# XuyangBai/D3Feat

Hardware: AMD Instinct MI355X
Metric: fragments/sec (30k-pt clouds) (higher is better)
Workload: dtype f32; 1 GPU; SURVEY §8d config #2: synthetic 3DMatch room fragment, 300k raw pts -> grid subsample 0.03 m (~29k pts per cloud) -> self-pair -> 5-level pyramid -> full KPFCNN forward (random-init weights (reference initialiser, seed 42), 14.1M params)...; points_per_cloud=29369, fragments_per_gpu=2141, parallelism=fragment-dp1, fragments_per_replay=12, engine_fallbacks=0, engine_isolated_replays=0

## Files before the change

### d3feat_amd/_lib.py

```python
import ctypes as C
import os

_HERE = os.path.dirname(os.path.abspath(__file__))
LIB_PATH = os.environ.get("D3FEAT_AMD_LIB") or os.path.join(_HERE, "lib", "libd3feat_amd.so")

D3F_OK = 0
ERRORS = {-1: "HIP runtime / kernel launch failure", -2: "workspace too small", -3: "invalid argument"}
ST_EMPTY_ELEMENT, ST_NEG_CELL, ST_KEY_RANGE, ST_HIT_OVERFLOW, ST_OUT_OVERFLOW, ST_KEY_WIDTH = 1, 2, 4, 8, 16, 32
PAD_NUM_SUPPORTS = -2147483648
NEIGHBOR_CAP = 1024
MAX_BATCH = 255
TOPK_MAX = 8192
PAIRS_KMAX = 1024
REPEAT_COUNTS_MAX = 16
MATCH_KMAX = 8192
VALIDATION_NMAX = 1024
SCENES_MAX = 256
GRID_RESET_MAX = 8
VP_INDEX_RANGE, VP_COUNT_RANGE = 1, 2

_vp, _sz, _i, _f = C.c_void_p, C.c_size_t, C.c_int, C.c_float

SIGNATURES = {
    "d3f_version": (_i, []),
    "d3f_trace_marker": (_i, [_i, _vp]),
    "d3f_pack_status": (_i, [_vp, _vp, _i, _vp, _i, _vp, _i, _vp, _i, _vp, _i, _i, _i, _vp]),
    "d3f_grid_subsample_workspace_bytes": (_sz, [_i, _i, _i, _i]),
    "d3f_batch_grid_subsample": (_i, [_vp, _i, _vp, _i, _f, _vp, _i, _vp, _i, _vp, _vp, _vp, _vp, _vp, _vp, _sz, _vp]),
    "d3f_batch_grid_subsample_async": (_i, [_vp, _i, _vp, _i, _f, _vp, _i, _i, _i, _vp, _vp, _vp, _sz, _vp]),
    "d3f_batch_grid_subsample_async_inplace": (_i, [_vp, _i, _vp, _i, _f, _vp, _i, _i, _vp, _vp, _vp, _sz, _vp]),
    "d3f_stack_self_pair": (_i, [_vp, _i, _vp, _i, _vp, _vp, _vp, _vp]),
    "d3f_radius_neighbors_workspace_bytes": (_sz, [_i, _i, _i]),
    "d3f_batch_radius_neighbors": (_i, [_vp, _i, _vp, _i, _vp, _vp, _i, _f, _vp, _i, _i, _i, _vp, _vp, _sz, _vp]),
    "d3f_neighbor_grid_bytes": (_sz, [_i, _i]),
    "d3f_neighbor_grid_order_offset": (_sz, [_i, _i]),
    "d3f_neighbor_grid_build": (_i, [_vp, _i, _vp, _i, _f, _vp, _sz, _vp]),
    "d3f_neighbor_grid_boxed_form": (_i, [_i, _i]),
    "d3f_geometry_reset": (_i, [_vp, _i, _vp, _vp, _vp, _vp, _i, _vp]),
    "d3f_neighbor_grid_build_boxed": (_i, [_vp, _i, _vp, _i, _f, _vp, _vp, _sz, _vp]),
    "d3f_stack_self_pair_boxed": (_i, [_vp, _i, _vp, _i, _vp, _vp, _vp, _vp, _vp, _vp]),
    "d3f_batch_grid_subsample_async_boxed": (_i, [_vp, _vp, _i, _vp, _i, _f, _vp, _i, _i, _i, _vp, _vp, _vp, _vp, _vp, _sz, _vp]),
    "d3f_neighbor_grid_search": (_i, [_vp, _sz, _i, _vp, _i, _vp, _i, _f, _i, _vp, _i, _i, _i, _i, _i, _f, _i, _vp, _vp]),
    "d3f_neighbor_grid_search_ordered": (_i, [_vp, _sz, _i, _vp, _i, _vp, _i, _f, _vp, _sz, _vp, _i, _i, _i, _i, _i, _f, _i, _vp, _vp]),
    "d3f_neighbor_grid_inv_offset": (_sz, [_i, _i]),
    "d3f_neighbor_grid_xyz_offset": (_sz, [_i, _i]),
    "d3f_row_positive": (_i, [_vp, _i, _i, _i, _vp, _vp, _i, _vp]),
    "d3f_kpconv_aggregate": (_i, [_vp, _i, _vp, _i, _vp, _i, _i, _vp, _i, _i, _vp, _vp, _i, _f, _i, _i, _vp, _vp, _vp, _vp,
                                  _vp, _i, _vp]),
    "d3f_kpconv_deform_aggregate": (_i, [_vp, _i, _vp, _i, _vp, _i, _i, _vp, _i, _i, _vp, _i, _f, _vp, _i, _i, _vp, _i, _f, _i, _i, _vp,
                                         _vp, _vp, _vp, _i, _vp]),
    "d3f_kpconv_fused_c1": (_i, [_vp, _i, _vp, _i, _vp, _i, _i, _vp, _i, _vp, _i, _f, _i, _i, _vp, _i, _vp, _vp, _vp, _i, _i,
                                 _f, _vp, _i, _vp, _vp, _vp, _i, _vp]),
    "d3f_kpconv_fused32": (_i, [_vp, _i, _vp, _i, _vp, _i, _i, _vp, _i, _vp, _vp, _i, _f, _i, _i, _vp, _vp, _vp, _vp, _i, _i, _f, _vp,
                                _i, _vp, _vp, _vp, _i, _vp]),
    "d3f_kpconv_fused_supported": (_i, [_i, _i, _i, _i, _i]),
    "d3f_kpconv_pack_weights": (_i, [_vp, _i, _i, _vp, _vp]),
    "d3f_kpconv_fused": (_i, [_vp, _i, _vp, _i, _vp, _i, _i, _vp, _i, _i, _vp, _vp, _i, _f, _i, _i, _vp, _i, _vp, _vp, _vp, _i, _i,
                              _f, _vp, _i, _vp, _vp, _vp, _i, _vp]),
    "d3f_kpconv_fused32_x3": (_i, [_vp, _i, _vp, _i, _vp, _i, _i, _vp, _i, _vp, _vp, _i, _f, _i, _i, _vp, _vp, _vp, _vp, _i, _i, _f, _vp,
                                   _i, _vp, _vp, _vp, _i, _vp]),
    "d3f_kpconv_packed_x3_bytes": (_sz, [_i, _i]),
    "d3f_kpconv_pack_weights_x3": (_i, [_vp, _i, _i, _vp, _vp]),
    "d3f_kpconv_fused_x3": (_i, [_vp, _i, _vp, _i, _vp, _i, _i, _vp, _i, _i, _vp, _vp, _i, _f, _i, _i, _vp, _i, _vp, _vp, _vp, _i, _i,
                                 _f, _vp, _i, _vp, _vp, _vp, _i, _vp]),
    "d3f_gemm_workspace_bytes": (_sz, [_i, _i, _i, _i]),
    "d3f_gemm_bf16_workspace_bytes": (_sz, [_i, _i, _i, _i]),
    "d3f_gemm_f32": (_i, [_vp, _i, _vp, _i, _vp, _i, _i, _i, _i, _vp, _vp, _vp, _vp, _i, _i, _f, _vp, _sz, _vp, _i, _vp]),
    "d3f_gemm_upsample_cat_f32": (_i, [_vp, _i, _i, _i, _vp, _i, _vp, _i, _i, _vp, _i, _vp, _i, _i, _i, _vp, _vp, _i, _f, _vp, _sz,
                                       _vp, _vp, _i, _vp]),
    "d3f_ind_max_pool": (_i, [_vp, _i, _i, _i, _vp, _i, _i, _i, _vp, _i, _vp, _vp, _vp, _vp, _i, _vp]),
    "d3f_closest_pool_cat": (_i, [_vp, _i, _i, _i, _vp, _i, _i, _vp, _i, _i, _vp, _i, _vp, _vp, _vp]),
    "d3f_affine_act": (_i, [_vp, _i, _i, _i, _vp, _vp, _vp, _i, _i, _f, _vp, _i, _vp, _vp]),
    "d3f_pack_descriptors": (_i, [_vp, _vp, _i, _i, _vp, _i, _vp, _i, _vp, _vp]),
    "d3f_pack_descriptors_to": (_i, [_vp, _vp, _i, _i, _vp, _i, _vp, _i, _vp, _vp, _i, _i, _i, _vp, _vp, _vp]),
    "d3f_topk_workspace_bytes": (_sz, [_i, _i, _i, _i]),
    "d3f_topk_records": (_i, [_vp, _i, _vp, _i, _i, _vp, _i, _i, _vp, _vp, _i, _i, _i, _vp, _i, _i, _vp, _i, _vp, _vp, _vp, _vp, _sz,
                              _vp]),
    "d3f_feature_nn_workspace_bytes": (_sz, [_i]),
    "d3f_feature_nn": (_i, [_vp, _i, _i, _vp, _i, _i, _i, _vp, _vp, _vp, _sz, _vp]),
    "d3f_mutual_matches_workspace_bytes": (_sz, [_i]),
    "d3f_mutual_matches": (_i, [_vp, _i, _vp, _i, _vp, _vp, _vp, _sz, _vp]),
    "d3f_ransac_hypotheses": (_i, [_vp, _i, _vp, _i, _vp, _i, _f, _f, C.c_uint64, C.c_uint64, _i, _vp, _vp, _vp]),
    "d3f_ransac_draw": (_i, [C.c_uint64, C.c_uint64, _i, _i]),
    "d3f_neighbor_grid_score": (_i, [_vp, _sz, _i, _vp, _i, _vp, _i, _f, _vp, _vp, _vp, _vp]),
    "d3f_register_pairs_workspace_bytes": (_sz, [_i, _i, _i, _i]),
    "d3f_register_pairs": (_i, [_vp, _i, _i, _i, _i, _vp, _vp, _i, _i, _f, _i, _f, _f, _i, _i, C.c_uint64, _vp, _f] + [_vp] * 11
                           + [_sz, _vp]),
    "d3f_repeatability_pairs": (_i, [_vp, _i, _i, _i, _vp, _vp, _i, _vp, _i, _vp, _vp, _i, _vp, _vp, _vp]),
    "d3f_match_pairs_workspace_bytes": (_sz, [_i, _vp, _i]),
    "d3f_match_pairs": (_i, [_vp, _i, _i, _i, _i, _vp, _vp, _i, _vp, _f, _vp, _i, _vp, _vp, _vp, _sz, _vp]),
    "d3f_register_pairs_counts_workspace_bytes": (_sz, [_i, _i, _i, _vp, _i, _i]),
    "d3f_register_pairs_counts": (_i, [_vp, _i, _i, _i, _i, _vp, _vp, _i, _vp, _i, _f, _i, _f, _f, _i, _i, C.c_uint64, _vp, _f] + [_vp] * 10
                                  + [_sz, _vp]),
    "d3f_overlap_pairs": (_i, [_vp, _sz, _i, _i, _vp, _i, _f, _vp, _vp, _i, _vp]),
    "d3f_validation_pairs_workspace_bytes": (_sz, [_i, _i]),
    "d3f_validation_pairs": (_i, [_vp, _i, _i, _vp, _i, _vp, _i, _i, _vp, _vp, _vp, _i, _vp, _i, _f, _i, _f, _f, _f, _f] + [_vp] * 5
                             + [_sz, _vp]),
    "d3f_loss_gradients_workspace_bytes": (_sz, [_i, _i, _i]),
    "d3f_loss_gradients": (_i, [_vp, _i, _i, _vp, _i, _vp, _i, _i, _vp, _vp, _vp, _i, _vp, _i, _f, _i, _f, _f, _f, _f, _i, _vp, _i, _vp, _i,
                                _vp, _vp, _vp, _sz, _vp]),
    "d3f_neighbor_transpose_workspace_bytes": (_sz, [_i, _i]),
    "d3f_neighbor_transpose": (_i, [_vp, _i, _i, _i, _vp, _i, _vp, _vp, _vp, _sz, _vp]),
    "d3f_detect_head_backward_workspace_bytes": (_sz, [_i, _i, _i]),
    "d3f_detect_head_backward": (_i, [_vp, _i, _i, _i, _vp, _i, _i, _vp, _vp, _i, _i, _vp, _vp, _vp, _i, _vp, _i, _vp, _i, _vp, _sz, _vp]),
    "d3f_pose_errors": (_i, [_vp, _vp, _i, _i, _vp, _vp, _vp, _vp, _vp, _vp]),
    "d3f_sanitize_descriptors": (_i, [_vp, _i, _i, _i, _i, _vp]),
    "d3f_matching_summary": (_i, [_vp, _vp, _vp, _i, _i, _vp, _i, _vp, _vp, _vp, _vp]),
    "d3f_registration_recall": (_i, [_vp, _i, _vp, _vp, _vp, _vp, _vp, _i, _i, _vp, _i, _vp, _vp, _vp, _vp, _vp]),
    "d3f_icp_pairs_workspace_bytes": (_sz, [_i, _i]),
    "d3f_icp_pairs": (_i, [_vp, _sz, _i, _vp, _i, _vp, _i, _vp, _vp, _i, _i] + [_vp] * 9 + [_sz, _vp]),
    "d3f_gemm_pack_bf16": (_i, [_vp, _i, _i, _i, _vp, _vp]),
    "d3f_gemm_pack_f32t": (_i, [_vp, _i, _i, _i, _vp, _vp]),
    "d3f_gemm_f32t": (_i, [_vp, _i, _i, _i, _vp, _i, _vp, _i, _i, _vp, _vp, _i, _i, _i, _vp, _vp, _vp, _vp, _i, _i, _f, _vp, _sz,
                           _vp, _vp, _i, _vp]),
    "d3f_gemm_x3_packed_bytes": (_sz, [_i, _i]),
    "d3f_gemm_pack_x3": (_i, [_vp, _i, _i, _i, _vp, _vp]),
    "d3f_gemm_x3_workspace_bytes": (_sz, [_i, _i, _i, _i]),
    "d3f_gemm_x3_plan": (_i, [_i, _i, _i, _i, _vp, _vp, _vp]),
    "d3f_gemm_x3_resident": (_i, [_i, _i, _i, _i]),
    "d3f_gemm_x3": (_i, [_vp, _i, _i, _i, _vp, _i, _vp, _i, _i, _vp, _vp, _i, _i, _i, _vp, _vp, _vp, _vp, _i, _i, _f, _vp, _sz,
                         _vp, _vp, _i, _vp]),
    "d3f_gemm_x3_gres": (_i, [_vp, _i, _i, _i, _vp, _i, _vp, _i, _i, _vp, _vp, _i, _i, _i, _vp, _vp, _vp, _vp, _i, _vp, _i, _i, _vp, _i, _f,
                              _vp, _sz, _vp, _vp, _i, _vp]),
    "d3f_gemm_bf16": (_i, [_vp, _i, _i, _i, _vp, _i, _vp, _i, _i, _vp, _vp, _i, _i, _i, _vp, _vp, _vp, _vp, _i, _i, _f, _vp, _sz,
                           _vp, _vp, _i, _i, _i, _vp]),
    "d3f_decode_xyz_records": (_i, [_vp, _i, _i, _i, _i, _i, _i, _i, _vp, _vp]),
    "d3f_detect_head": (_i, [_vp, _i, _i, _i, _vp, _i, _i, _vp, _vp, _i, _i, _vp, _i, _vp, _vp, _vp, _vp]),
}

_lib = None


class D3FeatLibraryError(RuntimeError):
    pass


def load():
    global _lib
    if _lib is not None:
        return _lib
    if not os.path.exists(LIB_PATH):
        raise D3FeatLibraryError(
            "d3feat_amd: %s not found -- the HIP extension is the only compute path. Build it with "
            "`python -c 'import __graft_entry__ as g; g.build()'` or `make -C d3feat_amd/csrc`." % LIB_PATH)
    lib = C.CDLL(LIB_PATH)
    for name, (res, args) in SIGNATURES.items():
        fn = getattr(lib, name)
        fn.restype = res
        fn.argtypes = args
    _lib = lib
    return lib


def check(rc, what):
    if rc != D3F_OK:
        raise D3FeatLibraryError("d3feat_amd.%s failed: %s (code %d)" % (what, ERRORS.get(rc, "unknown"), rc))
```

### d3feat_amd/csrc/gemm_common.h

```cpp
#pragma once
#include "common.h"
#include <type_traits>

typedef float f32x16 __attribute__((ext_vector_type(16)));

#define GM_BK 32

struct GemmGather {
    const int* gidx;
    int ld_gidx;
    int N1;
    const int* N1_dev;
    const float* A2;
    int lda2;
    int K1;
};

struct GemmEpi {
    const float* row_scale;
    const float* col_scale;
    const float* col_shift;
    const float* residual;
    int ldr;
    int leaky;
    float alpha;
    const int* ridx;
    int ld_ridx;
    int res_rows;
    const int* res_rows_dev;
};

__device__ __forceinline__ const float* gemm_residual_row(const GemmEpi& E, int m) {
    if (!E.ridx) return E.residual + (size_t)m * E.ldr;
    const int r = E.ridx[(size_t)m * E.ld_ridx];
    return (r >= 0 && r < d3f_dyn(E.res_rows, E.res_rows_dev)) ? E.residual + (size_t)r * E.ldr : nullptr;
}

__device__ __forceinline__ float gemm_epilogue(float v, int m, int n, const GemmEpi& E) {
    if (E.row_scale) v *= E.row_scale[m];
    if (E.col_scale) v *= E.col_scale[n];
    if (E.col_shift) v += E.col_shift[n];
    if (E.residual) v += E.residual[(size_t)m * E.ldr + n];
    if (E.leaky) v = v > 0.f ? v : v * E.alpha;
    return v;
}

__device__ __forceinline__ void gemm_tile_mfma(f32x16& acc, const float* as, const float* bs, int q0, int q1, int q2, int q3) {
    const int coff[4] = {q0, q1, q2, q3};
    float4 fa[4], fb[4];
#pragma unroll
    for (int q = 0; q < 4; ++q) {
        fa[q] = *(const float4*)&as[coff[q]];
        fb[q] = *(const float4*)&bs[coff[q]];
    }
    __builtin_amdgcn_sched_barrier(0);
#pragma unroll
    for (int q = 0; q < 4; ++q) {
#pragma unroll
        for (int e = 0; e < 4; ++e) {
            const float a = e == 0 ? fa[q].x : e == 1 ? fa[q].y : e == 2 ? fa[q].z : fa[q].w;
            const float b = e == 0 ? fb[q].x : e == 1 ? fb[q].y : e == 2 ? fb[q].z : fb[q].w;
            acc = __builtin_amdgcn_mfma_f32_32x32x2f32(b, a, acc, 0, 0, 0);
        }
    }
}

__global__ void __launch_bounds__(256)
gemm_splitk_reduce_kernel(const float* __restrict__ slab, int S, int M, int N, float* __restrict__ C, int ldc, GemmEpi E,
                          const int* __restrict__ M_dev, int res_bf16 = 0, int c_bf16 = 0) {
    const long long i = (long long)blockIdx.x * blockDim.x + threadIdx.x;
    if (i >= (long long)d3f_dyn(M, M_dev) * N) return;
    const int m = (int)(i / N), n = (int)(i % N);
    float v = 0.f;
    for (int s = 0; s < S; ++s) v += slab[((size_t)s * M + m) * N + n];
    if (res_bf16 && E.residual) {
        const float r = d3f_bf16_f32(((const unsigned short*)E.residual)[(size_t)m * E.ldr + n]);
        GemmEpi E2 = E;
        E2.residual = nullptr;
        E2.leaky = 0;
        v = gemm_epilogue(v, m, n, E2) + r;
        if (E.leaky) v = v > 0.f ? v : v * E.alpha;
    } else if (E.ridx && E.residual) {
        const float* rrow = gemm_residual_row(E, m);
        GemmEpi E2 = E;
        E2.residual = nullptr;
        E2.leaky = 0;
        v = gemm_epilogue(v, m, n, E2) + (rrow ? rrow[n] : 0.f);
        if (E.leaky) v = v > 0.f ? v : v * E.alpha;
    } else {
        v = gemm_epilogue(v, m, n, E);
    }
    if (c_bf16) ((unsigned short*)C)[(size_t)m * ldc + n] = (unsigned short)d3f_bf16_rne(v);
    else C[(size_t)m * ldc + n] = v;
}

static inline size_t gemm_slab_bytes(int S, int M, int N) { return S > 1 ? d3f_align((size_t)S * M * N * sizeof(float)) + 256 : 256; }

static inline int gemm_slab(int S, int M, int N, void* workspace, size_t workspace_bytes, float*& slab) {
    slab = nullptr;
    if (S > 1) {
        if (!workspace || workspace_bytes < (size_t)S * M * N * sizeof(float)) return D3F_ERR_WORKSPACE;
        slab = (float*)workspace;
    }
    return D3F_OK;
}

static inline void gemm_reduce(const float* slab, int S, int M, int N, float* C, int ldc, const GemmEpi& E, const int* M_dev,
                               hipStream_t stream, int res_bf16 = 0, int c_bf16 = 0) {
    if (S > 1)
        gemm_splitk_reduce_kernel<<<d3f_cdiv((long long)M * N, 256), 256, 0, stream>>>(slab, S, M, N, C, ldc, E, M_dev, res_bf16, c_bf16);
}

static inline int gemm_check_composite(bool f32_io, int kmul, unsigned a_mask, int M, int N, int N1, int C1, int C2, int lda, int ldc,
                                       int lds, int ldr, int ld_idx, const void* A, const void* W, const void* C, const int* idx,
                                       const void* skip, const void* residual, const float* col_scale, const float* col_shift,
                                       bool& empty) {
    const int q = f32_io ? 4 : 1;
    empty = false;
    if (M < 0 || N < 1 || N1 < 0 || C1 < 4 || C2 < 0 || (C1 % 4) || (C2 % 4) || (N % q) || lda < C1 || (lda % 4) || ldc < N || (ldc % q) ||
        (C2 > 0 && (lds < C2 || (lds % 4))) || (residual && (ldr < N || (ldr % q))) || (idx && ld_idx < 1) || (!idx && N1 < M))
        return D3F_ERR_ARG;
    if (((C1 + C2) % kmul) || (C2 > 0 && (C1 % kmul))) return D3F_ERR_ARG;
    empty = M == 0;
    if (empty) return D3F_OK;
    if (!A || !W || !C || (C2 > 0 && !skip) || ((uintptr_t)W & 15) || (((uintptr_t)A | (uintptr_t)skip) & a_mask)) return D3F_ERR_ARG;
    if (f32_io && (((uintptr_t)C | (uintptr_t)residual | (uintptr_t)col_scale | (uintptr_t)col_shift) & 15)) return D3F_ERR_ARG;
    return D3F_OK;
}

template <class F> static inline void gemm_with_epi(const GemmEpi& E, F&& f) {
    switch ((E.row_scale ? 1 : 0) | (E.residual ? 2 : 0)) {
    case 0: f(std::integral_constant<int, 0>{}); break;
    case 1: f(std::integral_constant<int, 1>{}); break;
    case 2: f(std::integral_constant<int, 2>{}); break;
    default: f(std::integral_constant<int, 3>{}); break;
    }
}

static inline void gemm_plan(int M, int N, int K, int M_hint, int& bm, int& bn, int& S, int& tps) {
    if (M_hint > 0 && M_hint < M) M = M_hint;
    auto blocks_of = [&](int m, int n) { return (long long)d3f_cdiv(M, m) * d3f_cdiv(N, n); };
    if (N <= 32) { bm = 128; bn = 32; }
    else { bm = 64; bn = 64; }
    const long long blocks = blocks_of(bm, bn);
    const int nt = d3f_cdiv(K, GM_BK);
    S = 1;
    if (blocks < 768 && nt > 16) {
        long long want = (1536 + blocks - 1) / blocks;
        long long maxs = nt / 8;
        S = (int)(want < maxs ? want : maxs);
        if (S > 64) S = 64;
        if (S < 1) S = 1;
    }
    tps = d3f_cdiv(nt, S);
    S = d3f_cdiv(nt, tps);
}
```

### d3feat_amd/csrc/gemm_f32.hip

```cpp
#include "gemm_common.h"
#include <cstdio>
#include <cstdlib>

#define GM_SA (GM_BK + 1)

template <int WM, int WN>
__global__ void __launch_bounds__(256)
gemm_f32_kernel(const float* __restrict__ A, int lda, const float* __restrict__ B, int ldb, float* __restrict__ C, int ldc,
                int M, int N, int K, int vecA, int vecB, int tiles_per_split, float* __restrict__ slab, GemmEpi E,
                const int* __restrict__ M_dev, GemmGather G) {
    constexpr int BM = 32 * WM, BN = 32 * WN;
    constexpr int A_F4 = BM * GM_BK / 4 / 256;
    constexpr int B_F4 = GM_BK * BN / 4 / 256;
    static_assert(WM * WN == 4 && A_F4 >= 1 && B_F4 >= 1, "tile shape");
    const int Mcap = M;
    M = d3f_dyn(M, M_dev);
    if ((int)(blockIdx.z * BM) >= M) return;
    __shared__ float As[2][BM * GM_SA];
    __shared__ __attribute__((aligned(16))) float Bs[2][GM_BK * BN];

    const int tid = threadIdx.x, lane = tid & 63, wave = tid >> 6;
    const int wm = wave / WN, wn = wave % WN;
    const int m0 = blockIdx.z * BM, n0 = blockIdx.x * BN;
    const int nt_all = (K + GM_BK - 1) / GM_BK;
// ... 381 lines not shown
    if (int rc = gemm_check_composite(true, 4, 15, M, N, N1, C1, C2, lda, ldc, lds, ldr, ld_idx, A, Wt, C, idx, skip, residual,
                                      col_scale, col_shift, empty))
        return rc;
    if (empty) return D3F_OK;
    const int Kp = (K + GD_BK - 1) / GD_BK * GD_BK;
    int bm, bn, S, tps;
    gemm_plan(M, N, K, M_hint, bm, bn, S, tps);
    float* slab;
    if (int rc = gemm_slab(S, M, N, workspace, workspace_bytes, slab)) return rc;
    GemmEpi E{row_scale, col_scale, col_shift, residual, ldr, leaky, alpha};
    GemmGather G{idx, ld_idx, N1, N1_dev, C2 > 0 ? skip : nullptr, lds, C1};
    static_assert((size_t)GD_STAGES * (128 + 32) * GD_BK * sizeof(float) <= 65536, "the ring needs an LDS opt-in (d3f_opt_in_lds)");
    const size_t lds_bytes = (size_t)GD_STAGES * (bm + bn) * GD_BK * sizeof(float);
    const long long items_cap = (long long)d3f_cdiv(N, bn) * S * d3f_cdiv(M, bm);
    const long long gsz = (items_cap + 7) / 8 * 8;
    if (gsz > 0x7fffffffll) return D3F_ERR_ARG;
    const dim3 grid((unsigned)gsz, 1, 1);
    gemm_with_epi(E, [&](auto epi) {
        constexpr int EPI = decltype(epi)::value;
        if (bn == 32) gemm_dma_kernel<4, 1, EPI><<<grid, 256, lds_bytes, stream>>>(A, lda, Wt, Kp, C, ldc, M, N, K, tps, S, slab, E, M_dev, G);
        else gemm_dma_kernel<2, 2, EPI><<<grid, 256, lds_bytes, stream>>>(A, lda, Wt, Kp, C, ldc, M, N, K, tps, S, slab, E, M_dev, G);
    });
    gemm_reduce(slab, S, M, N, C, ldc, E, M_dev, stream);
    D3F_LAUNCH_CHECK();
    return D3F_OK;
}

typedef __bf16 gb_bf16x8 __attribute__((ext_vector_type(8)));
#define GB_BK 32
#define GB_LS 40

__device__ __forceinline__ unsigned gb_pack2(float a, float b) { return d3f_bf16_rne(a) | (d3f_bf16_rne(b) << 16); }

__global__ void __launch_bounds__(256) gemm_pack_bf16_kernel(const float* __restrict__ B, int ldb, int K, int N, int Kp,
                                                             unsigned short* __restrict__ Wt) {
    const long long t = (long long)blockIdx.x * blockDim.x + threadIdx.x;
    if (t >= (long long)N * Kp) return;
    const int n = (int)(t / Kp), k = (int)(t % Kp);
    Wt[t] = (unsigned short)(k < K ? d3f_bf16_rne(B[(size_t)k * ldb + n]) : 0u);
}

extern "C" int d3f_gemm_pack_bf16(const float* B, int ldb, int K, int N, void* Wt, void* stream_) {
    hipStream_t stream = (hipStream_t)stream_;
    if (K < 1 || N < 1 || ldb < N || !B || !Wt) return D3F_ERR_ARG;
    const int Kp = (K + GB_BK - 1) / GB_BK * GB_BK;
    gemm_pack_bf16_kernel<<<d3f_cdiv((long long)N * Kp, 256), 256, 0, stream>>>(B, ldb, K, N, Kp, (unsigned short*)Wt);
    D3F_LAUNCH_CHECK();
    return D3F_OK;
}

template <bool ABF, bool CBF>
__global__ void __launch_bounds__(256)
gemm_bf16_kernel(const float* __restrict__ A, int lda, const unsigned short* __restrict__ Wt, int Kp, float* __restrict__ C,
                 int ldc, int M, int N, int K, int tiles_per_split, float* __restrict__ slab, GemmEpi E,
                 const int* __restrict__ M_dev, GemmGather G) {
    constexpr int BM = 64, BN = 64;
    const int Mcap = M;
    M = d3f_dyn(M, M_dev);
    if ((int)(blockIdx.z * BM) >= M) return;
    const unsigned gx_ = gridDim.x, gxy_ = gridDim.x * gridDim.y;
    const unsigned T_ = d3f_xcd_tile(blockIdx.x + gx_ * blockIdx.y + gxy_ * blockIdx.z, gxy_ * (unsigned)((M + BM - 1) / BM));
    const unsigned bz = T_ / gxy_, by = (T_ % gxy_) / gx_, bx = T_ % gx_;
    __shared__ __attribute__((aligned(16))) unsigned short As[2][BM * GB_LS];
    __shared__ __attribute__((aligned(16))) unsigned short Bs[2][BN * GB_LS];
    const int tid = threadIdx.x, lane = tid & 63, wave = tid >> 6;
    const int wm = wave >> 1, wn = wave & 1;
    const int m0 = bz * BM, n0 = bx * BN;
    const int nt_all = Kp / GB_BK;
    const int t_begin = by * tiles_per_split;
    const int t_end = min(nt_all, t_begin + tiles_per_split);
    int srow[2];
    {
        const int n1 = d3f_dyn(G.N1, G.N1_dev);
#pragma unroll
        for (int i = 0; i < 2; ++i) {
            const int gm = m0 + ((tid + i * 256) >> 3);
            int sr = gm < M ? gm : -1;
            if (G.gidx && sr >= 0) {
                sr = G.gidx[(size_t)gm * G.ld_gidx];
                if (sr < 0 || sr >= n1) sr = -1;
            }
            srow[i] = sr;
        }
    }
    const int brow = n0 + (tid >> 2);
    float4 ra[2];
    uint2 rh[2];
    uint4 rb;
    const unsigned short* Ah = (const unsigned short*)A;
    const unsigned short* A2h = (const unsigned short*)G.A2;
    auto load_tile = [&](int t) {
        const int k0 = t * GB_BK;
#pragma unroll
        for (int i = 0; i < 2; ++i) {
            const int e = tid + i * 256;
            const int gm = m0 + (e >> 3), k = k0 + ((e & 7) << 2);
            if (ABF) {
                uint2 v = make_uint2(0u, 0u);
                if (gm < M && k < K) {
                    if (G.A2 && k >= G.K1) v = *(const uint2*)(A2h + (size_t)gm * G.lda2 + (k - G.K1));
                    else if (srow[i] >= 0) v = *(const uint2*)(Ah + (size_t)srow[i] * lda + k);
                }
                rh[i] = v;
            } else {
                float4 v = make_float4(0.f, 0.f, 0.f, 0.f);
                if (gm < M && k < K) {
                    if (G.A2 && k >= G.K1) v = *(const float4*)(G.A2 + (size_t)gm * G.lda2 + (k - G.K1));
                    else if (srow[i] >= 0) v = *(const float4*)(A + (size_t)srow[i] * lda + k);
                }
                ra[i] = v;
            }
        }
        rb = (brow < N) ? *(const uint4*)(Wt + (size_t)brow * Kp + k0 + ((tid & 3) << 3)) : make_uint4(0u, 0u, 0u, 0u);
    };
    auto store_tile = [&](int buf) {
#pragma unroll
        for (int i = 0; i < 2; ++i) {
            const int e = tid + i * 256;
            const uint2 p = ABF ? rh[i] : make_uint2(gb_pack2(ra[i].x, ra[i].y), gb_pack2(ra[i].z, ra[i].w));
            *(uint2*)&As[buf][(e >> 3) * GB_LS + ((e & 7) << 2)] = p;
        }
        *(uint4*)&Bs[buf][(tid >> 2) * GB_LS + ((tid & 3) << 3)] = rb;
    };
    f32x16 acc;
#pragma unroll
    for (int r = 0; r < 16; ++r) acc[r] = 0.f;
    if (t_begin < t_end) {
        load_tile(t_begin);
        store_tile(0);
        __syncthreads();
        for (int t = t_begin; t < t_end; ++t) {
            const int buf = (t - t_begin) & 1;
            if (t + 1 < t_end) load_tile(t + 1);
            const unsigned short* ap = &As[buf][(32 * wm + (lane & 31)) * GB_LS + ((lane >> 5) << 3)];
            const unsigned short* bp = &Bs[buf][(32 * wn + (lane & 31)) * GB_LS + ((lane >> 5) << 3)];
            const uint4 a0 = *(const uint4*)ap, a1 = *(const uint4*)(ap + 16);
            const uint4 b0 = *(const uint4*)bp, b1 = *(const uint4*)(bp + 16);
            acc = __builtin_amdgcn_mfma_f32_32x32x16_bf16(__builtin_bit_cast(gb_bf16x8, a0), __builtin_bit_cast(gb_bf16x8, b0), acc, 0, 0, 0);
            acc = __builtin_amdgcn_mfma_f32_32x32x16_bf16(__builtin_bit_cast(gb_bf16x8, a1), __builtin_bit_cast(gb_bf16x8, b1), acc, 0, 0, 0);
            if (t + 1 < t_end) store_tile(buf ^ 1);
            __syncthreads();
        }
    }
    const int gn = n0 + 32 * wn + (lane & 31);
    if (gn >= N) return;
    float cs = 1.f, ch = 0.f;
    if (!slab) { cs = E.col_scale ? E.col_scale[gn] : 1.f; ch = E.col_shift ? E.col_shift[gn] : 0.f; }
#pragma unroll
    for (int r = 0; r < 16; ++r) {
        const int gm = m0 + 32 * wm + (r & 3) + 8 * (r >> 2) + 4 * (lane >> 5);
        if (gm >= M) continue;
        if (slab) { slab[((size_t)by * Mcap + gm) * N + gn] = acc[r]; continue; }
        float v = acc[r];
        if (E.row_scale) v *= E.row_scale[gm];
        v = v * cs + ch;
        if (E.residual)
            v += ABF ? d3f_bf16_f32(((const unsigned short*)E.residual)[(size_t)gm * E.ldr + gn]) : E.residual[(size_t)gm * E.ldr + gn];
        if (E.leaky) v = v > 0.f ? v : v * E.alpha;
        if (CBF) ((unsigned short*)C)[(size_t)gm * ldc + gn] = (unsigned short)d3f_bf16_rne(v);
        else C[(size_t)gm * ldc + gn] = v;
    }
}

static void gemm_bf16_split(int M, int N, int K, int M_hint, int& S, int& tps) {
    int bm, bn;
    gemm_plan(M, N > 32 ? N : 64, K, M_hint, bm, bn, S, tps);
    const int nt = ((K + GB_BK - 1) / GB_BK * GB_BK) / GB_BK;
    if (S > nt) S = nt;
    tps = d3f_cdiv(nt, S);
    S = d3f_cdiv(nt, tps);
}

extern "C" size_t d3f_gemm_bf16_workspace_bytes(int M, int N, int K, int M_hint) {
    if (M <= 0 || N <= 0 || K <= 0) return 256;
    int S, tps;
    gemm_bf16_split(M, N, K, M_hint, S, tps);
    return gemm_slab_bytes(S, M, N);
}

extern "C" int d3f_gemm_bf16(const void* A_, int N1, int lda, int C1, const int* idx, int ld_idx, const void* skip_, int lds,
                             int C2, const void* Wt, void* C_, int ldc, int M, int N, const float* row_scale,
                             const float* col_scale, const float* col_shift, const void* residual_, int ldr, int leaky,
                             float alpha, void* workspace, size_t workspace_bytes, const int* M_dev, const int* N1_dev,
                             int M_hint, int a_bf16, int c_bf16, void* stream_) {
    hipStream_t stream = (hipStream_t)stream_;
    const float* A = (const float*)A_;
    const float* skip = (const float*)skip_;
    const float* residual = (const float*)residual_;
    float* C = (float*)C_;
    const int K = C1 + C2;
    bool empty;
    if (int rc = gemm_check_composite(false, 4, a_bf16 ? 7 : 15, M, N, N1, C1, C2, lda, ldc, lds, ldr, ld_idx, A, Wt, C, idx, skip,
                                      residual, col_scale, col_shift, empty))
        return rc;
    if (empty) return D3F_OK;
    const int Kp = (K + GB_BK - 1) / GB_BK * GB_BK;
    int S, tps;
    gemm_bf16_split(M, N, K, M_hint, S, tps);
    float* slab;
    if (int rc = gemm_slab(S, M, N, workspace, workspace_bytes, slab)) return rc;
    if (d3f_cdiv(M, 64) > 65535) return D3F_ERR_ARG;
    GemmEpi E{row_scale, col_scale, col_shift, residual, ldr, leaky, alpha};
    GemmGather G{idx, ld_idx, N1, N1_dev, C2 > 0 ? skip : nullptr, lds, C1};
    dim3 grid(d3f_cdiv(N, 64), S, d3f_cdiv(M, 64));
#define D3F_GB(ABF_, CBF_) gemm_bf16_kernel<ABF_, CBF_><<<grid, 256, 0, stream>>>(A, lda, (const unsigned short*)Wt, Kp, C, ldc, M, N, K, tps, slab, E, M_dev, G)
    if (a_bf16) { if (c_bf16) D3F_GB(true, true); else D3F_GB(true, false); }
    else { if (c_bf16) D3F_GB(false, true); else D3F_GB(false, false); }
#undef D3F_GB
    gemm_reduce(slab, S, M, N, C, ldc, E, M_dev, stream, a_bf16, c_bf16);
    D3F_LAUNCH_CHECK();
    return D3F_OK;
}

#include "gemm_x3.h"

struct GemmX3Plan { int tn, waves, S, tps; };
static long long gemm_x3_cost(long long blocks, long long slots, int nt, int per_tile_x100, int& S) {
    long long best = -1;
    S = 1;
    for (int s = 1; s <= 64 && s * 4 <= nt; ++s) {
        const int t = d3f_cdiv(nt, s);
        if (d3f_cdiv(nt, t) != s) continue;
        const long long rounds = (blocks * s + slots - 1) / slots;
        const long long cost = rounds * (t + 12) * per_tile_x100 + (s > 1 ? 200ll * s : 0);
        if (best < 0 || cost < best) { best = cost; S = s; }
    }
    if (best < 0) best = ((blocks + slots - 1) / slots) * (nt + 12) * per_tile_x100;
    return best;
}
static GemmX3Plan gemm_x3_plan(int M, int N, int K, int M_hint) {
    if (M_hint > 0 && M_hint < M) M = M_hint;
    const int nt = K / GX_BK;
    GemmX3Plan p;
#ifdef D3F_GEMM_TUNING
    static const char* forced = getenv("D3F_X3_PLAN");
    if (forced) {
        int tn = 0, wv = 0, S = 0;
        if (sscanf(forced, "%d,%d,%d", &tn, &wv, &S) == 3 && ((tn == 1 && wv == 4) || (tn == 2 && wv == 4) || (tn == 4 && wv == 8)) && S >= 1 &&
            !(N <= 32 && tn != 1) && S * 4 <= (nt > 4 ? nt : 4)) {
            p.tn = tn; p.waves = wv; p.S = S < nt ? S : nt;
            p.tps = d3f_cdiv(nt, p.S);
            p.S = d3f_cdiv(nt, p.tps);
            return p;
        }
    }
#endif
    p.tn = N <= 32 ? 1 : 2;
    p.waves = 4;
    const long long c_small = gemm_x3_cost((long long)d3f_cdiv(M, 128) * d3f_cdiv(N, 32 * p.tn), 512, nt, 100, p.S);
    if (N >= 128) {
        int s_big;
        const long long c_big = gemm_x3_cost((long long)d3f_cdiv(M, 256) * d3f_cdiv(N, 128), 256, nt, 163, s_big);
        if (c_big < c_small) { p.tn = 4; p.waves = 8; p.S = s_big; }
    }
    p.tps = d3f_cdiv(nt, p.S);
    p.S = d3f_cdiv(nt, p.tps);
    return p;
}

extern "C" size_t d3f_gemm_x3_packed_bytes(int K, int N) {
    if (K < 1 || N < 1) return 0;
    return (size_t)d3f_cdiv(N, 32) * d3f_cdiv(K, GX_BK) * GX_CHUNK * sizeof(unsigned short);
}

extern "C" int d3f_gemm_pack_x3(const float* B, int ldb, int K, int N, void* Wx, void* stream_) {
    hipStream_t stream = (hipStream_t)stream_;
    if (K < 1 || N < 1 || ldb < N || !B || !Wx || ((uintptr_t)Wx & 15)) return D3F_ERR_ARG;
    const int nkt = d3f_cdiv(K, GX_BK);
    const long long total = (long long)d3f_cdiv(N, 32) * nkt * GX_CHUNK;
    gemm_pack_x3_kernel<<<d3f_cdiv(total, 256), 256, 0, stream>>>(B, ldb, K, N, nkt, total, (unsigned short*)Wx);
    D3F_LAUNCH_CHECK();
    return D3F_OK;
}

extern "C" int d3f_gemm_x3_plan(int M, int N, int K, int M_hint, int* rows, int* cols, int* slices) {
    if (M <= 0 || N <= 0 || K < GX_BK || (K % GX_BK)) return D3F_ERR_ARG;
    const GemmX3Plan p = gemm_x3_plan(M, N, K, M_hint);
    if (rows) *rows = 32 * p.waves;
    if (cols) *cols = 32 * p.tn;
    if (slices) *slices = p.S;
    return D3F_OK;
}

extern "C" size_t d3f_gemm_x3_workspace_bytes(int M, int N, int K, int M_hint) {
    if (M <= 0 || N <= 0 || K < GX_BK) return 256;
    const GemmX3Plan p = gemm_x3_plan(M, N, K, M_hint);
    return gemm_slab_bytes(p.S, M, N);
}

static size_t gemm_x3r_lds_bytes(int nkt, int NG) {
    return (size_t)nkt * NG * GX_CHUNK * sizeof(unsigned short) + GXR_PATCH_BYTES + GXR_EPI_BYTES;
}

extern "C" int d3f_gemm_x3_resident(int M, int N, int K, int M_hint) {
    if (N < 1 || K < GX_BK || (K % GX_BK)) return 0;
    const int NG = d3f_cdiv(N, 32), m_eff = (M_hint > 0 && M_hint < M) ? M_hint : M;
    return (NG == 1 || NG == 2 || NG == 4) && gemm_x3r_lds_bytes(K / GX_BK, NG) <= 160 * 1024 && m_eff >= 65536;
}

static int gemm_x3_run(const float* A, int N1, int lda, int C1, const int* idx, int ld_idx, const float* skip, int lds, int C2,
                       const void* Wx, float* C, int ldc, int M, int N, const float* row_scale, const float* col_scale,
                       const float* col_shift, const float* residual, int ldr, const int* res_idx, int ld_res_idx, int res_rows,
                       const int* res_rows_dev, int leaky, float alpha, void* workspace, size_t workspace_bytes, const int* M_dev,
                       const int* N1_dev, int M_hint, void* stream_) {
    hipStream_t stream = (hipStream_t)stream_;
    const int K = C1 + C2;
    bool empty;
    if (int rc = gemm_check_composite(true, GX_BK, 15, M, N, N1, C1, C2, lda, ldc, lds, ldr, ld_idx, A, Wx, C, idx, skip, residual,
                                      col_scale, col_shift, empty))
        return rc;
    if (res_idx && (ld_res_idx < 1 || res_rows < 0)) return D3F_ERR_ARG;
    if (empty) return D3F_OK;
    if (res_idx && !residual) return D3F_ERR_ARG;
    GemmEpi E{row_scale, col_scale, col_shift, residual, ldr, leaky, alpha, res_idx, ld_res_idx, res_rows, res_rows_dev};
    GemmGather G{idx, ld_idx, N1, N1_dev, C2 > 0 ? skip : nullptr, lds, C1};
    const int nkt = K / GX_BK, NG = d3f_cdiv(N, 32);
    if (!res_idx && d3f_gemm_x3_resident(M, N, K, M_hint)) {
        static std::atomic<int> cus_of[64];
        int dev = 0;
        if (hipGetDevice(&dev) != hipSuccess) return D3F_ERR_HIP;
        int cus = cus_of[dev & 63].load(std::memory_order_relaxed);
        if (!cus) {
            hipDeviceProp_t pr;
            if (hipGetDeviceProperties(&pr, dev) != hipSuccess) return D3F_ERR_HIP;
            cus = pr.multiProcessorCount > 0 ? pr.multiProcessorCount : 256;
            cus_of[dev & 63].store(cus, std::memory_order_relaxed);
        }
        static std::atomic<unsigned long long> lds_done{0};
        const void* const fns[3] = {(const void*)gemm_x3r_kernel<1>, (const void*)gemm_x3r_kernel<2>, (const void*)gemm_x3r_kernel<4>};
        if (d3f_opt_in_lds(lds_done, fns, 160 * 1024) != D3F_OK) return D3F_ERR_HIP;
        const int grid = std::min(cus, d3f_cdiv(d3f_cdiv(M, 32), 8));
#define D3F_GXR(TN_) gemm_x3r_kernel<TN_><<<grid, 512, gemm_x3r_lds_bytes(nkt, NG), stream>>>(A, lda, (const unsigned short*)Wx, nkt, C, ldc, M, N, E, M_dev, G)
        if (NG == 4) D3F_GXR(4);
        else if (NG == 2) D3F_GXR(2);
        else D3F_GXR(1);
#undef D3F_GXR
        D3F_LAUNCH_CHECK();
        return D3F_OK;
    }
    const GemmX3Plan pl = gemm_x3_plan(M, N, K, M_hint);
    const int S = pl.S, tps = pl.tps, bm = 32 * pl.waves;
    float* slab;
    if (int rc = gemm_slab(S, M, N, workspace, workspace_bytes, slab)) return rc;
    if (d3f_cdiv(M, bm) > 65535) return D3F_ERR_ARG;
    dim3 grid(d3f_cdiv(N, 32 * pl.tn), S, d3f_cdiv(M, bm));
#define D3F_GX(TN_, WV_) gemm_x3_kernel<TN_, WV_><<<grid, 64 * WV_, 0, stream>>>(A, lda, (const unsigned short*)Wx, nkt, NG, C, ldc, M, N, tps, slab, E, M_dev, G)
    if (pl.waves == 8) D3F_GX(4, 8);
    else if (pl.tn == 1) D3F_GX(1, 4);
    else D3F_GX(2, 4);
#undef D3F_GX
    gemm_reduce(slab, S, M, N, C, ldc, E, M_dev, stream);
    D3F_LAUNCH_CHECK();
    return D3F_OK;
}

extern "C" int d3f_gemm_x3(const float* A, int N1, int lda, int C1, const int* idx, int ld_idx, const float* skip, int lds, int C2,
                           const void* Wx, float* C, int ldc, int M, int N, const float* row_scale, const float* col_scale,
                           const float* col_shift, const float* residual, int ldr, int leaky, float alpha, void* workspace,
                           size_t workspace_bytes, const int* M_dev, const int* N1_dev, int M_hint, void* stream_) {
    return gemm_x3_run(A, N1, lda, C1, idx, ld_idx, skip, lds, C2, Wx, C, ldc, M, N, row_scale, col_scale, col_shift, residual, ldr,
                       nullptr, 0, 0, nullptr, leaky, alpha, workspace, workspace_bytes, M_dev, N1_dev, M_hint, stream_);
}

extern "C" int d3f_gemm_x3_gres(const float* A, int N1, int lda, int C1, const int* idx, int ld_idx, const float* skip, int lds, int C2,
                                const void* Wx, float* C, int ldc, int M, int N, const float* row_scale, const float* col_scale,
                                const float* col_shift, const float* residual, int ldr, const int* res_idx, int ld_res_idx,
                                int res_rows, const int* res_rows_dev, int leaky, float alpha, void* workspace, size_t workspace_bytes,
                                const int* M_dev, const int* N1_dev, int M_hint, void* stream_) {
    return gemm_x3_run(A, N1, lda, C1, idx, ld_idx, skip, lds, C2, Wx, C, ldc, M, N, row_scale, col_scale, col_shift, residual, ldr,
                       res_idx, ld_res_idx, res_rows, res_rows_dev, leaky, alpha, workspace, workspace_bytes, M_dev, N1_dev, M_hint,
                       stream_);
}
```

### d3feat_amd/csrc/gemm_x3.h

```cpp
#pragma once
#include "gemm_common.h"

#define GX_BK 32
#define GX_LS 40
#define GX_CHUNK (3 * 32 * GX_LS)

__device__ __forceinline__ unsigned gx_cvt_pk(float lo, float hi) {
    unsigned r;
    asm("v_cvt_pk_bf16_f32 %0, %1, %2" : "=v"(r) : "v"(lo), "v"(hi));
    return r;
}

typedef float gx_f4 __attribute__((ext_vector_type(4)));
__device__ __forceinline__ void gx_ld16(gx_f4& r, const void* p) { asm volatile("global_load_dwordx4 %0, %1, off" : "=v"(r) : "v"(p) : "memory"); }
template <int OFF> __device__ __forceinline__ void gx_ld16o(gx_f4& r, const void* p) {
    asm volatile("global_load_dwordx4 %0, %1, off offset:%2" : "=v"(r) : "v"(p), "n"(OFF) : "memory");
}

__device__ __forceinline__ float gx_sub(float a, float b) {
    float r;
    asm("v_sub_f32 %0, %1, %2" : "=v"(r) : "v"(a), "v"(b));
    return r;
}
__device__ __forceinline__ void gx_split8(const gx_f4& x0, const gx_f4& x1, uint4 (&pl)[3]) {
    const float v[8] = {x0[0], x0[1], x0[2], x0[3], x1[0], x1[1], x1[2], x1[3]};
    unsigned p[3][4];
#pragma unroll
    for (int i = 0; i < 4; ++i) {
        float a = v[2 * i], b = v[2 * i + 1];
        p[0][i] = gx_cvt_pk(a, b);
        a = gx_sub(a, __uint_as_float(p[0][i] << 16));
        b = gx_sub(b, __uint_as_float(p[0][i] & 0xffff0000u));
        p[1][i] = gx_cvt_pk(a, b);
        a = gx_sub(a, __uint_as_float(p[1][i] << 16));
        b = gx_sub(b, __uint_as_float(p[1][i] & 0xffff0000u));
        p[2][i] = gx_cvt_pk(a, b);
    }
#pragma unroll
    for (int s = 0; s < 3; ++s) pl[s] = make_uint4(p[s][0], p[s][1], p[s][2], p[s][3]);
}

__global__ void __launch_bounds__(256) gemm_pack_x3_kernel(const float* __restrict__ B, int ldb, int K, int N, int nkt, long long total,
                                                           unsigned short* __restrict__ Wx) {
    const long long t = (long long)blockIdx.x * blockDim.x + threadIdx.x;
    if (t >= total) return;
    const int kk = (int)(t % GX_LS);
    long long q = t / GX_LS;
    const int r = (int)(q % 32); q /= 32;
    const int p = (int)(q % 3); q /= 3;
    const int kt = (int)(q % nkt);
    const int ng = (int)(q / nkt);
    const int k = kt * GX_BK + kk, n = ng * 32 + r;
    unsigned out = 0u;
    if (kk < GX_BK && k < K && n < N) {
        float w = B[(size_t)k * ldb + n];
        unsigned h = d3f_bf16_rne(w);
        if (p > 0) { w -= __uint_as_float(h << 16); h = d3f_bf16_rne(w); }
        if (p > 1) { w -= __uint_as_float(h << 16); h = d3f_bf16_rne(w); }
        out = h;
    }
    Wx[t] = (unsigned short)out;
}

template <int NB, int STRIDE>
__device__ __forceinline__ void gx_dma_round(const void* sbase, unsigned dst, const unsigned (&vo)[4]) {
    unsigned keep;
    if constexpr (NB == 2)
        asm volatile("s_mov_b32 %0, m0\n\ts_mov_b32 m0, %2\n\ts_nop 0\n\tglobal_load_lds_dwordx4 %3, %1\n\t"
                     "s_add_u32 m0, m0, %5\n\ts_nop 0\n\tglobal_load_lds_dwordx4 %4, %1\n\ts_mov_b32 m0, %0"
                     : "=&s"(keep) : "s"(sbase), "s"(dst), "v"(vo[0]), "v"(vo[1]), "n"(STRIDE) : "memory", "scc");
    else if constexpr (NB == 4)
        asm volatile("s_mov_b32 %0, m0\n\ts_mov_b32 m0, %2\n\ts_nop 0\n\tglobal_load_lds_dwordx4 %3, %1\n\t"
                     "s_add_u32 m0, m0, %7\n\ts_nop 0\n\tglobal_load_lds_dwordx4 %4, %1\n\t"
                     "s_add_u32 m0, m0, %7\n\ts_nop 0\n\tglobal_load_lds_dwordx4 %5, %1\n\t"
                     "s_add_u32 m0, m0, %7\n\ts_nop 0\n\tglobal_load_lds_dwordx4 %6, %1\n\ts_mov_b32 m0, %0"
                     : "=&s"(keep) : "s"(sbase), "s"(dst), "v"(vo[0]), "v"(vo[1]), "v"(vo[2]), "v"(vo[3]), "n"(STRIDE) : "memory", "scc");
    else static_assert(NB < 0, "add the round");
}

template <int TN, int WAVES>
__global__ void __launch_bounds__(64 * WAVES) __attribute__((amdgpu_waves_per_eu(2, 2)))
gemm_x3_kernel(const float* __restrict__ A, int lda, const unsigned short* __restrict__ Wx, int nkt, int NG, float* __restrict__ C,
               int ldc, int M, int N, int tiles_per_split, float* __restrict__ slab, GemmEpi E, const int* __restrict__ M_dev,
               GemmGather G) {
    constexpr int BM = 32 * WAVES, BN = 32 * TN, NTH = 64 * WAVES;
    constexpr int NB = (480 * TN + NTH - 1) / NTH;
    constexpr int SB = NB * NTH * 16;
    constexpr int WAITN = 4 + NB;
    static_assert((TN == 1 || TN == 2 || TN == 4) && (WAVES == 4 || WAVES == 8), "tile shape");
    const int Mcap = M;
    M = d3f_dyn(M, M_dev);
    if ((int)(blockIdx.z * BM) >= M) return;
    const unsigned gx_ = gridDim.x, gxy_ = gridDim.x * gridDim.y;
    const unsigned T_ = d3f_xcd_tile(blockIdx.x + gx_ * blockIdx.y + gxy_ * blockIdx.z, gxy_ * (unsigned)((M + BM - 1) / BM));
    const unsigned bz = T_ / gxy_, by = (T_ % gxy_) / gx_, bx = T_ % gx_;
    __shared__ __attribute__((aligned(16))) unsigned char Bs[3 * SB];
    const int tid = threadIdx.x, lane = tid & 63, wave = tid >> 6;
    const int m0 = bz * BM, n0 = bx * BN;
    const int t_begin = by * tiles_per_split;
    const int t_end = min(nkt, t_begin + tiles_per_split);
    const int t_last = t_end - 1;

    const int gm_a = m0 + 32 * wave + (lane & 31);
    const float* arow = gd_zero_line;
    const float* a2row = gd_zero_line;
    unsigned amask = 0u, a2mask = 0u;
    if (gm_a < M) {
        int sr = gm_a;
        if (G.gidx) {
            const int n1 = d3f_dyn(G.N1, G.N1_dev);
            sr = G.gidx[(size_t)gm_a * G.ld_gidx];
            if (sr < 0 || sr >= n1) sr = -1;
        }
        if (sr >= 0) { arow = A + (size_t)sr * lda; amask = 0xffffffffu; }
        if (G.A2) { a2row = G.A2 + (size_t)gm_a * G.lda2; a2mask = 0xffffffffu; }
    }
    const int kofs = (lane >> 5) << 3;
    const int K1 = G.K1;
    const float* pa;
    unsigned astep;
    int treq = t_begin;
    auto a_rebase = [&](int t) {
        const bool first = t * GX_BK < K1;
        const unsigned msk = first ? amask : a2mask;
        pa = (first ? arow : a2row) + ((unsigned)((first ? t * GX_BK : t * GX_BK - K1) + kofs) & msk);
        astep = (unsigned)GX_BK & msk;
    };
    a_rebase(t_begin);

    unsigned wofs[4];
#pragma unroll
    for (int i = 0; i < 4; ++i) {
        const int e = tid + NTH * (i < NB ? i : 0);
        const int c = e / 480, o = e - 480 * c;
        const int ng = min((int)bx * TN + c, NG - 1);
        wofs[i] = (unsigned)ng * (unsigned)nkt * (unsigned)(GX_CHUNK * 2) + (unsigned)o * 16u;
    }
    const unsigned lds_wave = (unsigned)__builtin_amdgcn_readfirstlane(
        (int)((unsigned)(unsigned long long)(gd_lptr)Bs + (unsigned)wave * 1024u));

    gx_f4 rA0, rA1, rA2, rA3, rB0, rB1, rB2, rB3, rC0, rC1, rC2, rC3;
    uint4 ap0[2][3], ap1[2][3];
    auto request_w = [&](int t, int slot) {
        gx_dma_round<NB, WAVES * 1024>((const char*)Wx + (size_t)t * (GX_CHUNK * 2), lds_wave + (unsigned)slot * (unsigned)SB, wofs);
    };
    auto request_a = [&](gx_f4& r0, gx_f4& r1, gx_f4& r2, gx_f4& r3) {
        gx_ld16(r0, pa);
        gx_ld16o<16>(r1, pa);
        gx_ld16o<64>(r2, pa);
        gx_ld16o<80>(r3, pa);
        if (treq < t_last) {
            ++treq;
            if (treq * GX_BK == K1) a_rebase(treq);
            else pa += astep;
        }
    };

    f32x16 acc[TN];
#pragma unroll
    for (int j = 0; j < TN; ++j)
#pragma unroll
        for (int r = 0; r < 16; ++r) acc[j][r] = 0.f;

    auto tile = [&](int slot, const uint4 (&cur)[2][3], uint4 (&nxt)[2][3], const gx_f4& r0, const gx_f4& r1, const gx_f4& r2,
                    const gx_f4& r3) {
        const unsigned short* bp = (const unsigned short*)(Bs + slot * SB) + (lane & 31) * GX_LS + kofs;
        constexpr int NM = 12 * TN, NOPS = 88;
        constexpr int PA[2][6] = {{2, 1, 0, 1, 0, 0}, {0, 1, 0, 2, 1, 0}}, PB[2][6] = {{0, 1, 2, 0, 1, 0}, {2, 1, 1, 0, 0, 0}};
        uint4 b[TN][3];
#pragma unroll
        for (int j = 0; j < TN; ++j)
#pragma unroll
            for (int p = 0; p < 3; ++p) b[j][p] = *(const uint4*)(bp + j * GX_CHUNK + p * (32 * GX_LS));
        float x[16] = {r0[0], r0[1], r0[2], r0[3], r1[0], r1[1], r1[2], r1[3], r2[0], r2[1], r2[2], r2[3], r3[0], r3[1], r3[2], r3[3]};
        float hl[16];
        unsigned P[3][8];
        __builtin_amdgcn_sched_barrier(0);
#pragma unroll
        for (int m = 0; m < NM; ++m) {
            const int s = m / (6 * TN), prod = (m % (6 * TN)) / TN, j = m % TN;
            acc[j] = __builtin_amdgcn_mfma_f32_32x32x16_bf16(__builtin_bit_cast(gb_bf16x8, b[j][PB[s][prod]]),
                                                             __builtin_bit_cast(gb_bf16x8, cur[s][PA[s][prod]]), acc[j], 0, 0, 0);
            if (s == 0 && (prod == 2 || prod >= 4)) {
                const int p = prod == 2 ? 2 : prod == 4 ? 1 : 0;
                b[j][p] = *(const uint4*)(bp + j * GX_CHUNK + p * (32 * GX_LS) + 16);
            }
#pragma unroll
            for (int k = m * NOPS / NM; k < (m + 1) * NOPS / NM; ++k) {
                const int lvl = k < 8 ? 0 : k < 24 ? 1 : k < 40 ? 2 : k < 48 ? 3 : k < 64 ? 4 : k < 80 ? 5 : 6;
                if (lvl == 0) P[0][k] = gx_cvt_pk(x[2 * k], x[2 * k + 1]);
                else if (lvl == 3) P[1][k - 40] = gx_cvt_pk(x[2 * (k - 40)], x[2 * (k - 40) + 1]);
                else if (lvl == 6) P[2][k - 80] = gx_cvt_pk(x[2 * (k - 80)], x[2 * (k - 80) + 1]);
                else if (lvl == 1 || lvl == 4) {
                    const int e = k - (lvl == 1 ? 8 : 48);
                    const unsigned pk = P[lvl == 1 ? 0 : 1][e >> 1];
                    hl[e] = __uint_as_float((e & 1) ? (pk & 0xffff0000u) : (pk << 16));
                } else {
                    const int e = k - (lvl == 2 ? 24 : 64);
                    x[e] = gx_sub(x[e], hl[e]);
                }
            }
            __builtin_amdgcn_sched_barrier(0);
        }
#pragma unroll
        for (int s = 0; s < 2; ++s)
#pragma unroll
            for (int p = 0; p < 3; ++p) nxt[s][p] = make_uint4(P[p][4 * s], P[p][4 * s + 1], P[p][4 * s + 2], P[p][4 * s + 3]);
    };
    auto landed = [&](gx_f4& r0, gx_f4& r1, gx_f4& r2, gx_f4& r3) {
        if constexpr (WAITN == 6) asm volatile("s_waitcnt vmcnt(6)" : "+v"(r0), "+v"(r1), "+v"(r2), "+v"(r3) : : "memory");
        else asm volatile("s_waitcnt vmcnt(8)" : "+v"(r0), "+v"(r1), "+v"(r2), "+v"(r3) : : "memory");
        static_assert(WAITN == 6 || WAITN == 8, "wait count");
    };

    if (t_begin < t_end) {
        int wslot = 0, cslot = 0;
        auto next = [&](int sl) { return sl + 1 == 3 ? 0 : sl + 1; };
        request_w(t_begin, wslot); wslot = next(wslot);
        request_a(rA0, rA1, rA2, rA3);
        request_a(rB0, rB1, rB2, rB3);
        request_w(min(t_begin + 1, t_last), wslot); wslot = next(wslot);
        request_a(rC0, rC1, rC2, rC3);
        if constexpr (NB == 2) asm volatile("s_waitcnt vmcnt(10)" : "+v"(rA0), "+v"(rA1), "+v"(rA2), "+v"(rA3) : : "memory");
        else asm volatile("s_waitcnt vmcnt(12)" : "+v"(rA0), "+v"(rA1), "+v"(rA2), "+v"(rA3) : : "memory");
        gx_split8(rA0, rA1, ap0[0]);
        gx_split8(rA2, rA3, ap0[1]);
#define GX_STEP(I_, CUR_, NXT_, C0_, C1_, C2_, C3_, Q0_, Q1_, Q2_, Q3_)                                                          \
        if (t + I_ < t_end) {                                                                                                  \
            landed(C0_, C1_, C2_, C3_);                                                                                        \
            __syncthreads();                                                                                                   \
            request_w(min(t + I_ + 2, t_last), wslot); wslot = next(wslot);                                                    \
            request_a(Q0_, Q1_, Q2_, Q3_);                                                                                     \
            tile(cslot, CUR_, NXT_, C0_, C1_, C2_, C3_); cslot = next(cslot);                                                  \
        }
        for (int t = t_begin; t < t_end; t += 6) {
            GX_STEP(0, ap0, ap1, rB0, rB1, rB2, rB3, rA0, rA1, rA2, rA3)
            GX_STEP(1, ap1, ap0, rC0, rC1, rC2, rC3, rB0, rB1, rB2, rB3)
            GX_STEP(2, ap0, ap1, rA0, rA1, rA2, rA3, rC0, rC1, rC2, rC3)
            GX_STEP(3, ap1, ap0, rB0, rB1, rB2, rB3, rA0, rA1, rA2, rA3)
            GX_STEP(4, ap0, ap1, rC0, rC1, rC2, rC3, rB0, rB1, rB2, rB3)
            GX_STEP(5, ap1, ap0, rA0, rA1, rA2, rA3, rC0, rC1, rC2, rC3)
        }
#undef GX_STEP
        asm volatile("s_waitcnt vmcnt(0)" : "+v"(rA0), "+v"(rA1), "+v"(rA2), "+v"(rA3), "+v"(rB0), "+v"(rB1), "+v"(rB2), "+v"(rB3), "+v"(rC0),
                     "+v"(rC1), "+v"(rC2), "+v"(rC3) : : "memory");
    }
    __syncthreads();

    const bool mok = gm_a < M;
    float rs = 1.f;
    if (!slab && E.row_scale && mok) rs = E.row_scale[gm_a];
    float* dst = slab ? slab + ((size_t)by * Mcap + (mok ? gm_a : 0)) * N : C + (size_t)(mok ? gm_a : 0) * ldc;
    const float* rrow = (!slab && E.residual && mok) ? gemm_residual_row(E, gm_a) : nullptr;
    static_assert(3 * SB >= WAVES * 32 * 36 * 4, "the output patches must fit the ring");
    float* patch = (float*)Bs + wave * (32 * 36);
#pragma unroll
    for (int j = 0; j < TN; ++j) {
        if (!slab) {
#pragma unroll
            for (int q = 0; q < 4; ++q) {
                const int gn = n0 + 32 * j + 8 * q + 4 * (lane >> 5);
                float v[4] = {acc[j][4 * q], acc[j][4 * q + 1], acc[j][4 * q + 2], acc[j][4 * q + 3]};
                if (mok && gn < N) {
                    const float4 c4 = E.col_scale ? *(const float4*)&E.col_scale[gn] : make_float4(1.f, 1.f, 1.f, 1.f);
                    const float4 h4 = E.col_shift ? *(const float4*)&E.col_shift[gn] : make_float4(0.f, 0.f, 0.f, 0.f);
                    const float4 r4 = rrow ? *(const float4*)&rrow[gn] : make_float4(0.f, 0.f, 0.f, 0.f);
                    const float c[4] = {c4.x, c4.y, c4.z, c4.w}, h[4] = {h4.x, h4.y, h4.z, h4.w}, rr[4] = {r4.x, r4.y, r4.z, r4.w};
#pragma unroll
                    for (int e = 0; e < 4; ++e) {
                        float t = (v[e] * rs) * c[e] + h[e];
                        t += rr[e];
                        v[e] = (E.leaky && !(t > 0.f)) ? t * E.alpha : t;
                    }
                }
                *(float4*)&patch[(lane & 31) * 36 + 8 * q + 4 * (lane >> 5)] = make_float4(v[0], v[1], v[2], v[3]);
            }
            __builtin_amdgcn_fence(__ATOMIC_RELEASE, "wavefront");
            __builtin_amdgcn_wave_barrier();
            const int cc = n0 + 32 * j + 4 * (lane & 7);
#pragma unroll
            for (int i = 0; i < 4; ++i) {
                const int r = (lane >> 3) + 8 * i;
                const float4 o = *(const float4*)&patch[r * 36 + 4 * (lane & 7)];
                const int gm = m0 + 32 * wave + r;
                if (gm < M && cc < N) *(float4*)&C[(size_t)gm * ldc + cc] = o;
            }
            __builtin_amdgcn_fence(__ATOMIC_ACQUIRE, "wavefront");
            __builtin_amdgcn_wave_barrier();
            continue;
        }
#pragma unroll
        for (int q = 0; q < 4; ++q) {
            const int gn = n0 + 32 * j + 8 * q + 4 * (lane >> 5);
            if (!mok || gn >= N) continue;
            float v[4] = {acc[j][4 * q], acc[j][4 * q + 1], acc[j][4 * q + 2], acc[j][4 * q + 3]};
            if (!slab) {
                const float4 c4 = E.col_scale ? *(const float4*)&E.col_scale[gn] : make_float4(1.f, 1.f, 1.f, 1.f);
                const float4 h4 = E.col_shift ? *(const float4*)&E.col_shift[gn] : make_float4(0.f, 0.f, 0.f, 0.f);
                const float4 r4 = rrow ? *(const float4*)&rrow[gn] : make_float4(0.f, 0.f, 0.f, 0.f);
                const float c[4] = {c4.x, c4.y, c4.z, c4.w}, h[4] = {h4.x, h4.y, h4.z, h4.w}, rr[4] = {r4.x, r4.y, r4.z, r4.w};
#pragma unroll
                for (int e = 0; e < 4; ++e) {
                    float t = (v[e] * rs) * c[e] + h[e];
                    t += rr[e];
                    v[e] = (E.leaky && !(t > 0.f)) ? t * E.alpha : t;
                }
            }
            *(float4*)&dst[gn] = make_float4(v[0], v[1], v[2], v[3]);
        }
    }
}

#define GXR_PS 36
#define GXR_PATCH_BYTES (8 * 32 * GXR_PS * 4)
#define GXR_EPI_BYTES (2 * 128 * 4)
template <int TN>
__global__ void __launch_bounds__(512) __attribute__((amdgpu_waves_per_eu(2, 2)))
gemm_x3r_kernel(const float* __restrict__ A, int lda, const unsigned short* __restrict__ Wx, int nkt, float* __restrict__ C, int ldc,
                int M, int N, GemmEpi E, const int* __restrict__ M_dev, GemmGather G) {
    extern __shared__ __attribute__((aligned(16))) unsigned char gxr_w[];
    static_assert(TN == 1 || TN == 2 || TN == 4, "column groups per row tile");
    M = d3f_dyn(M, M_dev);
    const int tid = threadIdx.x, lane = tid & 63, wave = tid >> 6;
    {
        const int total = nkt * TN * 480;
        const uint4* src = (const uint4*)Wx;
        uint4* dst = (uint4*)gxr_w;
        for (int e = tid; e < total; e += 512) {
            const int c = e / 480, o = e - 480 * c;
            const int kt = c / TN, j = c - kt * TN;
            dst[e] = src[(size_t)(j * nkt + kt) * 480 + o];
        }
        float* ep = (float*)(gxr_w + (size_t)nkt * TN * (GX_CHUNK * 2) + GXR_PATCH_BYTES);
        for (int c = tid; c < 32 * TN; c += 512) {
            ep[c] = (E.col_scale && c < N) ? E.col_scale[c] : 1.f;
            ep[32 * TN + c] = (E.col_shift && c < N) ? E.col_shift[c] : 0.f;
        }
    }
    __syncthreads();
    const float* ep_scale = (const float*)(gxr_w + (size_t)nkt * TN * (GX_CHUNK * 2) + GXR_PATCH_BYTES);
    const float* ep_shift = ep_scale + 32 * TN;
    const int ntiles = (M + 31) >> 5;
    auto kofs_now = [&]() -> int {
        unsigned l;
        asm volatile("v_mbcnt_lo_u32_b32 %0, -1, 0\n\tv_mbcnt_hi_u32_b32 %0, -1, %0" : "=v"(l));
        return (int)((l >> 5) << 3);
    };
    const int K1 = G.K1;
    const int n1 = G.gidx ? d3f_dyn(G.N1, G.N1_dev) : 0;
    const int tstride = 8 * (int)gridDim.x;
    const int rt0 = wave * (int)gridDim.x + (int)blockIdx.x;
    if (rt0 >= ntiles) return;
    const int ntl = (ntiles - rt0 + tstride - 1) / tstride;
    const int total = ntl * nkt;
    int rq_tile = rt0, rq_kt = 0;
    const float* arow;
    const float* a2row;
    unsigned amask, a2mask;
    const float* pa;
    unsigned astep;
    auto a_rebase = [&](int t) {
        const bool first = t * GX_BK < K1;
        const unsigned msk = first ? amask : a2mask;
        pa = (first ? arow : a2row) + ((unsigned)((first ? t * GX_BK : t * GX_BK - K1) + kofs_now()) & msk);
        astep = (unsigned)GX_BK & msk;
    };
    auto rq_rows = [&](int rt) {
        const int gm = rt * 32 + (lane & 31);
        arow = gd_zero_line; a2row = gd_zero_line; amask = 0u; a2mask = 0u;
        if (rt < ntiles && gm < M) {
            int sr = gm;
            if (G.gidx) {
                sr = G.gidx[(size_t)gm * G.ld_gidx];
                if (sr < 0 || sr >= n1) sr = -1;
            }
            if (sr >= 0) { arow = A + (size_t)sr * lda; amask = 0xffffffffu; }
            if (G.A2) { a2row = G.A2 + (size_t)gm * G.lda2; a2mask = 0xffffffffu; }
        }
        a_rebase(0);
    };
    rq_rows(rq_tile);
    gx_f4 rA0, rA1, rA2, rA3, rB0, rB1, rB2, rB3, rC0, rC1, rC2, rC3;
    uint4 ap0[2][3], ap1[2][3];
    auto request_a = [&](gx_f4& r0, gx_f4& r1, gx_f4& r2, gx_f4& r3) {
        gx_ld16(r0, pa);
        gx_ld16o<16>(r1, pa);
        gx_ld16o<64>(r2, pa);
        gx_ld16o<80>(r3, pa);
        if (++rq_kt == nkt) {
            rq_kt = 0;
            rq_tile += tstride;
            rq_rows(rq_tile);
        } else if (rq_kt * GX_BK == K1) a_rebase(rq_kt);
        else pa += astep;
    };
    f32x16 acc[TN];
#pragma unroll
    for (int j = 0; j < TN; ++j)
#pragma unroll
        for (int r = 0; r < 16; ++r) acc[j][r] = 0.f;
    auto tile = [&](int kt, const uint4 (&cur)[2][3], uint4 (&nxt)[2][3], const gx_f4& r0, const gx_f4& r1, const gx_f4& r2,
                    const gx_f4& r3) {
        const unsigned short* bp = (const unsigned short*)gxr_w + (size_t)kt * (TN * GX_CHUNK) + (lane & 31) * GX_LS + kofs_now();
        constexpr int NM = 12 * TN, NOPS = 88;
        constexpr int PA[2][6] = {{2, 1, 0, 1, 0, 0}, {0, 1, 0, 2, 1, 0}}, PB[2][6] = {{0, 1, 2, 0, 1, 0}, {2, 1, 1, 0, 0, 0}};
        uint4 b[TN][3];
#pragma unroll
        for (int j = 0; j < TN; ++j)
#pragma unroll
            for (int p = 0; p < 3; ++p) b[j][p] = *(const uint4*)(bp + j * GX_CHUNK + p * (32 * GX_LS));
        float x[16] = {r0[0], r0[1], r0[2], r0[3], r1[0], r1[1], r1[2], r1[3], r2[0], r2[1], r2[2], r2[3], r3[0], r3[1], r3[2], r3[3]};
        float hl[16];
        unsigned P[3][8];
        __builtin_amdgcn_sched_barrier(0);
#pragma unroll
        for (int m = 0; m < NM; ++m) {
            const int s = m / (6 * TN), prod = (m % (6 * TN)) / TN, j = m % TN;
            acc[j] = __builtin_amdgcn_mfma_f32_32x32x16_bf16(__builtin_bit_cast(gb_bf16x8, b[j][PB[s][prod]]),
                                                             __builtin_bit_cast(gb_bf16x8, cur[s][PA[s][prod]]), acc[j], 0, 0, 0);
            if (s == 0 && (prod == 2 || prod >= 4)) {
                const int p = prod == 2 ? 2 : prod == 4 ? 1 : 0;
                b[j][p] = *(const uint4*)(bp + j * GX_CHUNK + p * (32 * GX_LS) + 16);
            }
#pragma unroll
            for (int k = m * NOPS / NM; k < (m + 1) * NOPS / NM; ++k) {
                const int lvl = k < 8 ? 0 : k < 24 ? 1 : k < 40 ? 2 : k < 48 ? 3 : k < 64 ? 4 : k < 80 ? 5 : 6;
                if (lvl == 0) P[0][k] = gx_cvt_pk(x[2 * k], x[2 * k + 1]);
                else if (lvl == 3) P[1][k - 40] = gx_cvt_pk(x[2 * (k - 40)], x[2 * (k - 40) + 1]);
                else if (lvl == 6) P[2][k - 80] = gx_cvt_pk(x[2 * (k - 80)], x[2 * (k - 80) + 1]);
                else if (lvl == 1 || lvl == 4) {
                    const int e = k - (lvl == 1 ? 8 : 48);
                    const unsigned pk = P[lvl == 1 ? 0 : 1][e >> 1];
                    hl[e] = __uint_as_float((e & 1) ? (pk & 0xffff0000u) : (pk << 16));
                } else {
                    const int e = k - (lvl == 2 ? 24 : 64);
                    x[e] = gx_sub(x[e], hl[e]);
                }
            }
            __builtin_amdgcn_sched_barrier(0);
        }
#pragma unroll
        for (int s = 0; s < 2; ++s)
#pragma unroll
            for (int p = 0; p < 3; ++p) nxt[s][p] = make_uint4(P[p][4 * s], P[p][4 * s + 1], P[p][4 * s + 2], P[p][4 * s + 3]);
    };
    int c_tile = rt0, c_kt = 0;
    float* patch = (float*)(gxr_w + (size_t)nkt * TN * (GX_CHUNK * 2)) + wave * (32 * GXR_PS);
    auto finish_tile = [&]() {
        const int gm_a = c_tile * 32 + (lane & 31);
        const bool mok = gm_a < M;
        float rs = 1.f;
        if (E.row_scale && mok) rs = E.row_scale[gm_a];
#pragma unroll
        for (int j = 0; j < TN; ++j) {
#pragma unroll
            for (int q = 0; q < 4; ++q) {
                const int gn = 32 * j + 8 * q + 4 * (lane >> 5);
                float v[4] = {acc[j][4 * q], acc[j][4 * q + 1], acc[j][4 * q + 2], acc[j][4 * q + 3]};
                if (mok && gn < N) {
                    const float4 c4 = *(const float4*)&ep_scale[gn];
                    const float4 h4 = *(const float4*)&ep_shift[gn];
                    const float4 r4 = E.residual ? *(const float4*)&E.residual[(size_t)gm_a * E.ldr + gn] : make_float4(0.f, 0.f, 0.f, 0.f);
                    const float c[4] = {c4.x, c4.y, c4.z, c4.w}, h[4] = {h4.x, h4.y, h4.z, h4.w}, rr[4] = {r4.x, r4.y, r4.z, r4.w};
#pragma unroll
                    for (int e = 0; e < 4; ++e) {
                        float tt = (v[e] * rs) * c[e] + h[e];
                        tt += rr[e];
                        v[e] = (E.leaky && !(tt > 0.f)) ? tt * E.alpha : tt;
                    }
                }
                *(float4*)&patch[(lane & 31) * GXR_PS + 8 * q + 4 * (lane >> 5)] = make_float4(v[0], v[1], v[2], v[3]);
                acc[j][4 * q] = acc[j][4 * q + 1] = acc[j][4 * q + 2] = acc[j][4 * q + 3] = 0.f;
            }
            __builtin_amdgcn_fence(__ATOMIC_RELEASE, "wavefront");
            __builtin_amdgcn_wave_barrier();
            const int cc = 32 * j + 4 * (lane & 7);
#pragma unroll
            for (int i = 0; i < 4; ++i) {
                const int r = (lane >> 3) + 8 * i;
                const float4 o = *(const float4*)&patch[r * GXR_PS + 4 * (lane & 7)];
                const int gm = c_tile * 32 + r;
                if (gm < M && cc < N) *(float4*)&C[(size_t)gm * ldc + cc] = o;
            }
            __builtin_amdgcn_fence(__ATOMIC_ACQUIRE, "wavefront");
            __builtin_amdgcn_wave_barrier();
        }
        c_tile += tstride;
    };
    auto landed = [&](gx_f4& r0, gx_f4& r1, gx_f4& r2, gx_f4& r3) {
        asm volatile("s_waitcnt vmcnt(4)" : "+v"(r0), "+v"(r1), "+v"(r2), "+v"(r3) : : "memory");
    };
    request_a(rA0, rA1, rA2, rA3);
    request_a(rB0, rB1, rB2, rB3);
    request_a(rC0, rC1, rC2, rC3);
    asm volatile("s_waitcnt vmcnt(8)" : "+v"(rA0), "+v"(rA1), "+v"(rA2), "+v"(rA3) : : "memory");
    gx_split8(rA0, rA1, ap0[0]);
    gx_split8(rA2, rA3, ap0[1]);
#define GXR_STEP(I_, CUR_, NXT_, C0_, C1_, C2_, C3_, Q0_, Q1_, Q2_, Q3_)                                                         \
    if (it + I_ < total) {                                                                                                     \
        landed(C0_, C1_, C2_, C3_);                                                                                            \
        request_a(Q0_, Q1_, Q2_, Q3_);                                                                                         \
        tile(c_kt, CUR_, NXT_, C0_, C1_, C2_, C3_);                                                                            \
        if (++c_kt == nkt) { c_kt = 0; finish_tile(); }                                                                        \
    }
    for (int it = 0; it < total; it += 6) {
        GXR_STEP(0, ap0, ap1, rB0, rB1, rB2, rB3, rA0, rA1, rA2, rA3)
        GXR_STEP(1, ap1, ap0, rC0, rC1, rC2, rC3, rB0, rB1, rB2, rB3)
        GXR_STEP(2, ap0, ap1, rA0, rA1, rA2, rA3, rC0, rC1, rC2, rC3)
        GXR_STEP(3, ap1, ap0, rB0, rB1, rB2, rB3, rA0, rA1, rA2, rA3)
        GXR_STEP(4, ap0, ap1, rC0, rC1, rC2, rC3, rB0, rB1, rB2, rB3)
        GXR_STEP(5, ap1, ap0, rA0, rA1, rA2, rA3, rC0, rC1, rC2, rC3)
    }
#undef GXR_STEP
    asm volatile("s_waitcnt vmcnt(0)" : "+v"(rA0), "+v"(rA1), "+v"(rA2), "+v"(rA3), "+v"(rB0), "+v"(rB1), "+v"(rB2), "+v"(rB3), "+v"(rC0),
                 "+v"(rC1), "+v"(rC2), "+v"(rC3) : : "memory");
}
```

### d3feat_amd/kernels/convolution_ops.py

```python
import numpy as np
import torch

from .. import ops
from .kernel_points import create_kernel_points



def unary_convolution(features, K_values, epilogue=None):
    return ops.gemm(features, K_values, **(epilogue or {}))


def KPConv(query_points, support_points, neighbors_indices, features, K_values, fixed='center', KP_extent=1.0,
           KP_influence='linear', aggregation_mode='sum', K_points=None, epilogue=None):
    K_radius = 1.5 * KP_extent
    num_kpoints = int(K_values.shape[0])
    points_dim = int(query_points.shape[1])
    if K_points is None:
        K_points = create_kernel_points(K_radius, num_kpoints, num_kernels=1, dimension=points_dim, fixed=fixed)
        K_points = K_points.reshape((num_kpoints, points_dim)).astype(np.float32)
    return KPConv_ops(query_points, support_points, neighbors_indices, features, K_points, K_values, KP_extent,
                      KP_influence, aggregation_mode, epilogue=epilogue)


def KPConv_ops(query_points, support_points, neighbors_indices, features, K_points, K_values, KP_extent, KP_influence,
               aggregation_mode, epilogue=None):
    if KP_influence not in ('constant', 'linear', 'gaussian'):
        raise ValueError('Unknown influence function type (config.KP_influence)')
    if aggregation_mode not in ('closest', 'sum'):
        raise ValueError("Unknown convolution mode. Should be 'closest' or 'sum'")
    num_kp, cin, cout = K_values.shape
    if features.shape[1] != cin:
        raise ValueError('KPConv: features have %d channels, K_values expects %d' % (features.shape[1], cin))
    def _u24(rows, ld, lim=31):
        return rows < (1 << 24) and ld < (1 << 24) and rows * ld < (1 << lim)
    fused_ok = _u24(int(query_points.shape[0]), int(neighbors_indices.stride(0))) and \
        _u24(int(features.shape[0]), int(features.stride(0)), 30)
    if cin == 1 and cout <= 256:
        return ops.kpconv_fused_c1(query_points, support_points, neighbors_indices, features, K_points, K_values,
                                   KP_extent, KP_influence, aggregation_mode, **(epilogue or {}))
    if fused_ok and cin == 32 and cout == 32 and features.stride(0) % 4 == 0 and features.data_ptr() % 16 == 0:
        return ops.kpconv_fused32(query_points, support_points, neighbors_indices, features, K_points, K_values, KP_extent,
                                  KP_influence, aggregation_mode, **(epilogue or {}))
    if fused_ok and features.stride(0) % 4 == 0 and features.data_ptr() % 16 == 0 and \
            ops.kpconv_fused_supported(cin, cout, num_kp, KP_influence, aggregation_mode):
        return ops.kpconv_fused(query_points, support_points, neighbors_indices, features, K_points, K_values, KP_extent,
                                KP_influence, aggregation_mode, **(epilogue or {}))
    wf, inv_cnt = ops.kpconv_aggregate(query_points, support_points, neighbors_indices, features, K_points, KP_extent,
                                       KP_influence, aggregation_mode)
    return ops.gemm(wf, K_values.reshape(num_kp * cin, cout), row_scale=inv_cnt, **(epilogue or {}))


def KPConv_deformable(query_points, support_points, neighbors_indices, features, K_values, fixed='center', KP_extent=1.0,
                      KP_influence='linear', aggregation_mode='sum', modulated=False, K_points=None, offset_weights=None,
                      offset_bias=None, epilogue=None):
    if KP_influence not in ('constant', 'linear', 'gaussian'):
        raise ValueError('Unknown influence function type (config.KP_influence)')
    if aggregation_mode not in ('closest', 'sum'):
        raise ValueError("Unknown convolution mode. Should be 'closest' or 'sum'")
    K_radius = 1.5 * KP_extent
    num_kpoints, cin = int(K_values.shape[0]), int(K_values.shape[1])
    points_dim = int(query_points.shape[1])
    if K_points is None:
        K_points = create_kernel_points(K_radius, num_kpoints, num_kernels=1, dimension=points_dim, fixed=fixed)
        K_points = K_points.reshape((num_kpoints, points_dim)).astype(np.float32)
    offset_dim = (points_dim + 1 if modulated else points_dim) * num_kpoints
    if offset_weights is None:
        offset_weights = torch.zeros((num_kpoints, cin, offset_dim), dtype=torch.float32, device=features.device)
    if offset_bias is None:
        offset_bias = torch.zeros((offset_dim,), dtype=torch.float32, device=features.device)
    return ops.kpconv_deformable(query_points, support_points, neighbors_indices, features, K_points, K_values, offset_weights,
                                 offset_bias, KP_extent, KP_influence, aggregation_mode, modulated, **(epilogue or {}))


def KPConv_deform_ops(query_points, support_points, neighbors_indices, features, K_points, offsets, modulations, K_values, KP_extent,
                      KP_influence, mode, epilogue=None):
    if KP_influence not in ('constant', 'linear', 'gaussian'):
        raise ValueError('Unknown influence function type (config.KP_influence)')
    if mode not in ('closest', 'sum'):
        raise ValueError("Unknown convolution mode. Should be 'closest' or 'sum'")
    num_kp, cin, cout = K_values.shape
    if features.shape[1] != cin:
        raise ValueError('KPConv_deformable: features have %d channels, K_values expects %d' % (features.shape[1], cin))
    wf = ops.kpconv_deform_aggregate(query_points, support_points, neighbors_indices, features, K_points, offsets, KP_extent,
                                     KP_influence, mode, modulations=modulations)
    return ops.gemm(wf, K_values.reshape(num_kp * cin, cout), **(epilogue or {}))
```

### d3feat_amd/models/network_blocks.py

```python
import contextlib

import numpy as np

from .. import ops
from ..kernels import convolution_ops as conv_ops
from ..kernels.kernel_points import create_kernel_points

_STORE = None


@contextlib.contextmanager
def use_variables(store):
    global _STORE
    prev, _STORE = _STORE, store
    try:
        yield store
    finally:
        _STORE = prev


def _vs():
    if _STORE is None:
        raise RuntimeError('no VariableStore active: wrap the call in network_blocks.use_variables(store)')
    return _STORE


def variable_scope(name):
    return _vs().variable_scope(name)



def weight_variable(shape):
    vs = _vs()
    return vs.tensor(vs.weight_variable(shape))


def ind_max_pool(x, inds):
    return ops.ind_max_pool(x, inds)


def closest_pool(x, inds):
    return ops.closest_pool_cat(x, inds)


def _bn(channels, use_batch_norm=True):
    vs = _vs()
    if use_batch_norm:
        return vs.folded_bn(vs.batch_norm_variables(channels))
    name = vs.get('offset', (channels,), lambda: np.zeros(channels))
    return None, vs.tensor(name)


def batch_norm(x, use_batch_norm=True, momentum=0.99, training=False):
    if training:
        raise NotImplementedError('d3feat_amd implements the inference path only (training=False)')
    scale, shift = _bn(int(x.shape[1]), use_batch_norm)
    return ops.affine_act(x, scale, shift)


def leaky_relu(features, alpha=0.2):
    return ops.affine_act(features, leaky=True, alpha=alpha)


def _epilogue(channels, config, leaky, residual=None):
    scale, shift = _bn(channels, config.use_batch_norm)
    return dict(col_scale=scale, col_shift=shift, residual=residual, leaky=leaky, alpha=0.2)


def _kernel_points(config, extent):
    vs = _vs()
    k = config.num_kernel_points

    def init():
        pts = create_kernel_points(1.5 * extent, k, num_kernels=1, dimension=3, fixed=config.fixed_kernel_points,
                                   rng=vs.rng)
        return pts.reshape((k, 3))
    name = vs.get('kernel_points', (k, 3), init)
    return vs.values[name]


def KPConv(query_points, support_points, neighbors_indices, features, K_values, radius, config, epilogue=None):
    extent = config.KP_extent * radius / config.density_parameter
    return conv_ops.KPConv(query_points, support_points, neighbors_indices, features, K_values,
                           fixed=config.fixed_kernel_points, KP_extent=extent, KP_influence=config.KP_influence,
                           aggregation_mode=config.convolution_mode, K_points=_kernel_points(config, extent),
                           epilogue=epilogue)


def KPConv_deformable(query_points, support_points, neighbors_indices, features, K_values, radius, config, epilogue=None):
    extent = config.KP_extent * radius / config.density_parameter
    K_points = _kernel_points(config, extent)
    vs = _vs()
    k, cin = int(K_values.shape[0]), int(K_values.shape[1])
    offset_dim = (4 if config.modulated else 3) * k
    w0 = vs.tensor(vs.get('offset_conv_weights', (k, cin, offset_dim), lambda: np.zeros((k, cin, offset_dim))))
    b0 = vs.tensor(vs.get('offset_conv_bias', (offset_dim,), lambda: np.zeros(offset_dim)))
    return conv_ops.KPConv_deformable(query_points, support_points, neighbors_indices, features, K_values,
                                      fixed=config.fixed_kernel_points, KP_extent=extent, KP_influence=config.KP_influence,
                                      aggregation_mode=config.convolution_mode, modulated=config.modulated, K_points=K_points,
                                      offset_weights=w0, offset_bias=b0, epilogue=epilogue)


def _check_inference(training):
    if training:
        raise NotImplementedError('d3feat_amd implements the inference path only (training=False)')



def last_unary_block(layer_ind, inputs, features, radius, fdim, config, training):
    w = weight_variable([int(features.shape[1]), 32])
    with ops.f32_output():
        return conv_ops.unary_convolution(features, w)


def unary_block(layer_ind, inputs, features, radius, fdim, config, training):
    _check_inference(training)
    if isinstance(features, ops.UpsampleCat):
        vs = _vs()
        w = vs.weight_variable([int(features.shape[1]), fdim])
        if ops.upsample_split_ok(features, fdim):
            if config.use_batch_norm:
                w1, w2, shift = vs.split_decoder(w, vs.batch_norm_variables(fdim), int(features.x.shape[1]))
            else:
                (w1, w2, _), shift = vs.split_decoder(w, None, int(features.x.shape[1])), _bn(fdim, False)[1]
            return ops.gemm_upsample_split(features, w1, w2, col_shift=shift, leaky=True, alpha=0.2)
        e = _epilogue(fdim, config, True)
        return ops.gemm_upsample_cat(features, vs.tensor(w), col_scale=e['col_scale'], col_shift=e['col_shift'], leaky=True, alpha=0.2)
    w = weight_variable([int(features.shape[1]), fdim])
    return conv_ops.unary_convolution(features, w, epilogue=_epilogue(fdim, config, True))


def simple_block(layer_ind, inputs, features, radius, fdim, config, training):
    _check_inference(training)
    w = weight_variable([config.num_kernel_points, int(features.shape[1]), fdim])
    return KPConv(inputs['points'][layer_ind], inputs['points'][layer_ind], inputs['neighbors'][layer_ind], features, w,
                  radius, config, epilogue=_epilogue(fdim, config, True))


def _resnetb(layer_ind, inputs, features, radius, fdim, config, strided, deformable=False):
    cin = int(features.shape[1])
    with variable_scope('conv1'):
        w = weight_variable([cin, fdim // 2])
        x = conv_ops.unary_convolution(features, w, epilogue=_epilogue(fdim // 2, config, True))
    with variable_scope('conv2'):
        w = weight_variable([config.num_kernel_points, fdim // 2, fdim // 2])
        if strided:
            q, s, nb = inputs['points'][layer_ind + 1], inputs['points'][layer_ind], inputs['pools'][layer_ind]
        else:
            q, s, nb = inputs['points'][layer_ind], inputs['points'][layer_ind], inputs['neighbors'][layer_ind]
        x = (KPConv_deformable if deformable else KPConv)(q, s, nb, x, w, radius, config, epilogue=_epilogue(fdim // 2, config, True))
    with variable_scope('conv3'):
        vs = _vs()
        w3 = vs.weight_variable([fdim // 2, 2 * fdim])
        bn3 = vs.batch_norm_variables(2 * fdim) if config.use_batch_norm else None
    with variable_scope('shortcut'):
        shortcut = ind_max_pool(features, inputs['pools'][layer_ind]) if strided else features
        need_sc = int(shortcut.shape[1]) != 2 * fdim
        fuse = need_sc and config.use_batch_norm and (fdim // 2) % 4 == 0
        sc_w = sc_bn = None
        if need_sc:
            vs = _vs()
            sc_w = vs.weight_variable([int(shortcut.shape[1]), 2 * fdim])
            if fuse:
                sc_bn = vs.batch_norm_variables(2 * fdim)
            else:
                shortcut = conv_ops.unary_convolution(shortcut, vs.tensor(sc_w), epilogue=_epilogue(2 * fdim, config, False))
    with variable_scope('conv3'):
        vs = _vs()
        if fuse:
            W, shift = vs.stacked_branches(w3, bn3, sc_w, sc_bn)
            return ops.gemm_cat2(x, shortcut, W, col_shift=shift, leaky=True, alpha=0.2)
        return conv_ops.unary_convolution(x, vs.tensor(w3), epilogue=_epilogue(2 * fdim, config, True, residual=shortcut))


def resnetb_block(layer_ind, inputs, features, radius, fdim, config, training):
    _check_inference(training)
    return _resnetb(layer_ind, inputs, features, radius, fdim, config, False)


def resnetb_strided_block(layer_ind, inputs, features, radius, fdim, config, training):
    _check_inference(training)
    return _resnetb(layer_ind, inputs, features, radius, fdim, config, True)


def resnetb_deformable_block(layer_ind, inputs, features, radius, fdim, config, training):
    _check_inference(training)
    return _resnetb(layer_ind, inputs, features, radius, fdim, config, False, deformable=True)


def resnetb_deformable_strided_block(layer_ind, inputs, features, radius, fdim, config, training):
    _check_inference(training)
    return _resnetb(layer_ind, inputs, features, radius, fdim, config, True, deformable=True)


def nearest_upsample_block(layer_ind, inputs, features, radius, fdim, config, training):
    with variable_scope('nearest_upsample'):
        return closest_pool(features, inputs['upsamples'][layer_ind - 1])


def _materialized(block_fn):
    def wrapped(layer_ind, inputs, features, radius, fdim, config, training):
        if isinstance(features, ops.UpsampleCat):
            features = features.materialize()
        return block_fn(layer_ind, inputs, features, radius, fdim, config, training)
    wrapped.__name__ = block_fn.__name__
    wrapped.__doc__ = block_fn.__doc__
    return wrapped


def get_block_ops(block_name):
    table = {'unary': unary_block, 'last_unary': last_unary_block, 'simple': simple_block, 'resnetb': resnetb_block,
             'resnetb_strided': resnetb_strided_block, 'resnetb_deformable': resnetb_deformable_block,
             'resnetb_deformable_strided': resnetb_deformable_strided_block, 'nearest_upsample': nearest_upsample_block}
    if block_name in table:
        return table[block_name] if block_name == 'unary' else _materialized(table[block_name])
    known_unsupported = ('simple_strided', 'resnet', 'resnetb_light', 'inception_deformable',
                         'resnetb_light_strided', 'inception_deformable_strided', 'vgg',
                         'max_pool', 'max_pool_wide', 'global_average', 'simple_upsample', 'resnetb_upsample')
    if block_name in known_unsupported:
        raise NotImplementedError('block "%s" is not used by any released D3Feat model and is not implemented'
                                  % block_name)
    raise ValueError('Unknown block name in the architecture definition : ' + block_name)


def assemble_CNN_blocks(inputs, config, dropout_prob):
    r = config.first_subsampling_dl * config.density_parameter
    layer = 0
    fdim = config.first_features_dim
    features = inputs['features']
    F = []
    training = dropout_prob < 0.99
    block_in_layer = 0
    for block in config.architecture:
        if any(tmp in block for tmp in ('pool', 'strided', 'upsample', 'global')):
            F += [features]
        if 'upsample' in block:
            break
        with variable_scope('layer_{:d}/{:s}_{:d}'.format(layer, block.replace('_deformable', ''), block_in_layer)):
            features = get_block_ops(block)(layer, inputs, features, r, fdim, config, training)
        block_in_layer += 1
        if 'pool' in block or 'strided' in block:
            layer += 1
            r *= 2
            fdim *= 2
            block_in_layer = 0
        if 'global' in block:
            F += [features]
    return F
```

### d3feat_amd/ops.py

```python
import ctypes

import os

import numpy as np
import torch

from . import _lib

_WS = {}

PROFILE = None


class _timed:
    def __init__(self, name, info, device):
        self.on = PROFILE is not None
        self.name, self.info, self.device = name, info, device

    def __enter__(self):
        if self.on:
            self.start = torch.cuda.Event(enable_timing=True)
            self.end = torch.cuda.Event(enable_timing=True)
            self.start.record(torch.cuda.current_stream(self.device))
        return self
# ... 258 lines not shown

    def box(self, level):
        return self.boxes[level]

    def reset(self):
        import ctypes
        lib = _lib.load()
        ks = [k for k, on in enumerate(self.boxed) if on]
        n = len(ks)
        grids = (ctypes.c_void_p * max(n, 1))(*[self.mems[k].data_ptr() for k in ks])
        nbytes = (ctypes.c_size_t * max(n, 1))(*[self.nbytes[k] for k in ks])
        rows = (ctypes.c_int * max(n, 1))(*[self.rows[k] for k in ks])
        Bs = (ctypes.c_int * max(n, 1))(*([self.B] * n))
        rc = lib.d3f_geometry_reset(self.boxes.data_ptr(), self.boxes.numel() // 6, ctypes.addressof(grids), ctypes.addressof(nbytes),
                                    ctypes.addressof(rows), ctypes.addressof(Bs), n, _stream(self.boxes.device))
        _lib.check(rc, "geometry_reset")


class NeighborGrid:

    def __init__(self, supports, s_lens, radius, chain=None, level=0):
        lib = _lib.load()
        if chain is not None and chain.boxed[level]:
            self._init_boxed(lib, supports, s_lens, radius, chain, level)
            self._views(lib)
            return
        self.supports = _tag(_req(supports, torch.float32, "supports", 2).contiguous(), supports)
        dev = self.supports.device
        self.Ns = self.supports.shape[0]
        self.s_lens = as_lens(s_lens, dev)
        self.B = self.s_lens.numel()
        self.radius = float(radius)
        self.nbytes = lib.d3f_neighbor_grid_bytes(self.Ns, self.B)
        self.mem = torch.empty((self.nbytes,), dtype=torch.uint8, device=dev)
        with _timed("nb_grid_build", dict(Ns=self.Ns), dev):
            rc = lib.d3f_neighbor_grid_build(self.supports.data_ptr(), self.Ns, self.s_lens.data_ptr(), self.B, self.radius,
                                             self.mem.data_ptr(), self.nbytes, _stream(dev))
        _lib.check(rc, "neighbor_grid_build")
        self._views(lib)

    def _init_boxed(self, lib, supports, s_lens, radius, chain, level):
        self.supports = _tag(_req(supports, torch.float32, "supports", 2).contiguous(), supports)
        dev = self.supports.device
        self.Ns = self.supports.shape[0]
        self.s_lens = as_lens(s_lens, dev)
        self.B = self.s_lens.numel()
        self.radius = float(radius)
        if self.Ns != chain.rows[level] or self.B != chain.B:
            raise ValueError("grid chain level %d was laid out for %d rows / %d clouds, not %d / %d"
                             % (level, chain.rows[level], chain.B, self.Ns, self.B))
        self.nbytes, self.mem = chain.nbytes[level], chain.mems[level]
        self.form = chain.forms[level]
        with _timed("nb_grid_build", dict(Ns=self.Ns), dev):
            rc = lib.d3f_neighbor_grid_build_boxed(self.supports.data_ptr(), self.Ns, self.s_lens.data_ptr(), self.B, self.radius,
                                                   chain.box(level).data_ptr(), self.mem.data_ptr(), self.nbytes, _stream(dev))
        _lib.check(rc, "neighbor_grid_build_boxed")

    def _views(self, lib):
        dev = self.supports.device
        off = lib.d3f_neighbor_grid_order_offset(self.Ns, self.B)
        self.order = self.mem[off: off + 4 * max(self.Ns, 1)].view(torch.int32)
        off = lib.d3f_neighbor_grid_inv_offset(self.Ns, self.B)
        self.inv = self.mem[off: off + 4 * max(self.Ns, 1)].view(torch.int32)
        off = lib.d3f_neighbor_grid_xyz_offset(self.Ns, self.B)
        self.xyz = self.mem[off: off + 12 * max(self.Ns, 1)].view(torch.float32).view(-1, 3)
        for a in ("n_dev", "n_hint"):
            if getattr(self.supports, a, None) is not None:
                setattr(self.xyz, a, getattr(self.supports, a))

    def search(self, queries, q_lens, width, ld=None, pad_value=None, cap=192, first_only=False, out=None, status=None,
               reset_status=True, want_kmax=True, nn_hint=0.0, query_grid=None, internal=False):
        lib = _lib.load()
        queries = _req(queries, torch.float32, "queries", 2).contiguous()
        dev = queries.device
        Nq = queries.shape[0]
        ql = as_lens(q_lens, dev)
        if ql.numel() != self.B:
            raise ValueError("q_batches and s_batches must have the same number of elements")
        ld = int(ld if ld is not None else width)
        if out is None:
            out = torch.empty((Nq, ld), dtype=torch.int32, device=dev)
        if status is None:
            status = torch.empty((2,), dtype=torch.int32, device=dev)
        same = 1 if (queries.data_ptr() == self.supports.data_ptr() and Nq == self.Ns) else 0
        if pad_value is None:
            pad_value = _lib.PAD_NUM_SUPPORTS if getattr(self.supports, "n_dev", None) is not None else self.Ns
        if query_grid is not None:
            if query_grid.Ns != Nq or query_grid.B != self.B or query_grid.supports.data_ptr() != queries.data_ptr():
                raise ValueError("query_grid was not built over these queries")
            with _timed("nb_search", dict(Nq=Nq, Ns=self.Ns, width=int(width), first_only=int(bool(first_only))), dev):
                rc = lib.d3f_neighbor_grid_search_ordered(self.mem.data_ptr(), self.nbytes, self.Ns, queries.data_ptr(), Nq, ql.data_ptr(),
                                                          self.B, self.radius, query_grid.mem.data_ptr(), query_grid.nbytes,
                                                          out.data_ptr(), ld, int(width), int(pad_value), int(cap),
                                                          1 if first_only else 0, float(nn_hint),
                                                          (1 if reset_status else 0) | (0 if want_kmax else 2) | (4 if internal else 0),
                                                          status.data_ptr(), _stream(dev))
            _lib.check(rc, "neighbor_grid_search_ordered")
            o = getattr(queries, "order", None)
            if o is not None and not internal:
                out.order = o
            return _tag(out, queries), status
        if internal:
            raise ValueError("internal numbering needs the queries' grid")
        with _timed("nb_search", dict(Nq=Nq, Ns=self.Ns, width=int(width), first_only=int(bool(first_only))), dev):
            rc = lib.d3f_neighbor_grid_search(self.mem.data_ptr(), self.nbytes, self.Ns, queries.data_ptr(), Nq,
                                              ql.data_ptr(), self.B, self.radius, same, out.data_ptr(), ld, int(width),
                                              int(pad_value), int(cap),
                                              1 if first_only else 0, float(nn_hint),
                                              (1 if reset_status else 0) | (0 if want_kmax else 2),
                                              status.data_ptr(),
                                              _stream(dev))
        _lib.check(rc, "neighbor_grid_search")
        o = getattr(queries, "order", None)
        if o is not None:
            out.order = o
        return _tag(out, queries), status


def batch_radius_neighbors(queries, supports, q_lens, s_lens, radius, width, ld=None, out=None, pad_value=None, cap=192,
                           first_only=False):
    grid = NeighborGrid(supports, s_lens, radius)
    return grid.search(queries, q_lens, width, ld=ld, pad_value=pad_value, cap=cap, first_only=first_only, out=out)


class StackGroups:

    def __init__(self, group=0):
        self.group = int(group)


_KP_HOST = {}


def _kp_host(K_points):
    if isinstance(K_points, torch.Tensor):
        key = (K_points.data_ptr(), K_points._version, tuple(K_points.shape))
        hit = _KP_HOST.get(key)
        if hit is None:
            if len(_KP_HOST) > 256:
                _KP_HOST.clear()
            hit = _KP_HOST[key] = (K_points, np.ascontiguousarray(K_points.detach().cpu().numpy(), dtype=np.float32))
        return hit[1]
    return np.ascontiguousarray(K_points, dtype=np.float32)


_INFLUENCE = {"constant": 0, "linear": 1, "gaussian": 2}
_AGGREGATION = {"sum": 0, "closest": 1}


BF16_CONTRACTION = False


BF16_FEATURES = False
F32_OUTPUT = False


class bf16_contraction:

    def __init__(self, on=True, features=False):
        self.on, self.features = bool(on), bool(on) and bool(features)

    def __enter__(self):
        global BF16_CONTRACTION, BF16_FEATURES
        self.prev, BF16_CONTRACTION = BF16_CONTRACTION, self.on
        self.prevf, BF16_FEATURES = BF16_FEATURES, self.features
        return self

    def __exit__(self, *exc):
        global BF16_CONTRACTION, BF16_FEATURES
        BF16_CONTRACTION, BF16_FEATURES = self.prev, self.prevf
        return False


class f32_output:

    def __enter__(self):
        global F32_OUTPUT
        self.prev, F32_OUTPUT = F32_OUTPUT, True
        return self

    def __exit__(self, *exc):
        global F32_OUTPUT
        F32_OUTPUT = self.prev
        return False


def _feat(t, name, ndim=None):
    if isinstance(t, torch.Tensor) and t.dtype == torch.bfloat16:
        return _req(t, torch.bfloat16, name, ndim)
    return _req(t, torch.float32, name, ndim)


def _h(t):
    return 1 if (t is not None and t.dtype == torch.bfloat16) else 0


def _out_dtype():
    return torch.bfloat16 if (BF16_CONTRACTION and BF16_FEATURES and not F32_OUTPUT) else torch.float32


def _packed_on_tensor(W, slot, make):
    base = W._base if W._base is not None else W
    store = getattr(base, slot, None)
    if store is None:
        store = {}
        setattr(base, slot, store)
    key = (W.storage_offset(), tuple(W.shape), tuple(W.stride()))
    hit = store.get(key)
    if hit is None:
        hit = store[key] = [base._version, make(None)]
    elif hit[0] != base._version:
        make(hit[1])
        hit[0] = base._version
    return hit[1]


def refresh_packed_weights(tensors):
    n = 0
    for t in tensors:
        if not isinstance(t, torch.Tensor):
            continue
        base = t._base if t._base is not None else t
        for slot, fn in _PACKERS:
            for (off, shape, strides), hit in list((getattr(base, slot, None) or {}).items()):
                if hit[0] != base._version:
                    fn(base.as_strided(shape, strides, off))
                    n += 1
    return n


def _packed_weights(W, slot, alloc, pack, what):
    def make(t):
        K, N = W.shape
        if t is None:
            t = alloc(K, N)
        _lib.check(pack(W.data_ptr(), int(W.stride(0)), K, N, t.data_ptr(), _stream(W.device)), what)
        return t
    return _packed_on_tensor(W, slot, make)


def packed_bf16_weights(W):
    return _packed_weights(W, "_d3f_bf16t", lambda K, N: torch.empty((N, (K + 31) // 32 * 32), dtype=torch.int16, device=W.device),
                           _lib.load().d3f_gemm_pack_bf16, "gemm_pack_bf16")


def packed_f32t_weights(W):
    return _packed_weights(W, "_d3f_f32t", lambda K, N: torch.empty((N, (K + 31) // 32 * 32), dtype=torch.float32, device=W.device),
                           _lib.load().d3f_gemm_pack_f32t, "gemm_pack_f32t")


GEMM_X3 = os.environ.get("D3F_GEMM_X3", "1") != "0"


def packed_x3_weights(W):
    lib = _lib.load()
    return _packed_weights(W, "_d3f_x3", lambda K, N: torch.empty((int(lib.d3f_gemm_x3_packed_bytes(K, N)) // 2,), dtype=torch.int16,
                                                                  device=W.device), lib.d3f_gemm_pack_x3, "gemm_pack_x3")


X3_MAX_ROWS = 65535 * 128


def _x3_resident(M, N, K, hint):
    return bool(_lib.load().d3f_gemm_x3_resident(M, N, K, hint))


def _x3_ok(C1, C2, N, rows=0):
    fits = GEMM_X3 and (C1 + C2) % 32 == 0 and (C2 == 0 or C1 % 32 == 0)
    return fits and (N > 32 or _x3_resident(rows, N, C1 + C2, 0))


def _route(M, plain, bf16, bf16_ok, f32t_ok, x3, resident):
    if bf16 and bf16_ok:
        return "d3f_gemm_bf16", "gemm_bf16"
    if not f32t_ok:
        return ("d3f_gemm_f32" if plain else "d3f_gemm_upsample_cat_f32"), "gemm_f32"
    if x3 and M <= X3_MAX_ROWS:
        return "d3f_gemm_x3", "gemm_x3r" if resident else "gemm_x3"
    return "d3f_gemm_f32t", "gemm_f32"


def _f32t_ok(N, ldc, out, residual, ldr, vectors, *operands):
    if N % 4 or ldc % 4 or out.data_ptr() % 16:
        return False
    if residual is not None and (ldr % 4 or residual.data_ptr() % 16):
        return False
    if any(v is not None and v.data_ptr() % 16 for v in vectors):
        return False
    for t, ld, cols in operands:
        if t is not None and (cols % 4 or ld % 4 or t.data_ptr() % 16 or cols < 4):
            return False
    return True


def _bf16_ok(*operands):
    for t, ld, cols in operands:
        if t is None:
            continue
        if cols % 4 or ld % 4 or t.data_ptr() % (8 if t.dtype == torch.bfloat16 else 16):
            return False
    return True


def _contract(what, A, N1, lda, C1, idx, ld_idx, skip, lds, C2, W, ldb, out, ldc, m_dev, n1_dev, hint, row_scale=None, col_scale=None,
              col_shift=None, residual=None, ldr=0, leaky=False, alpha=0.2):
    lib = _lib.load()
    (M, N), K, dev = out.shape, C1 + C2, out.device
    operands = ((A, lda, C1), (skip, lds, C2))
    entry, name = _route(M, idx is None and skip is None, BF16_CONTRACTION,
                         K >= 4 and ldc == N and W.is_contiguous() and _bf16_ok(*operands),
                         W.is_contiguous() and _f32t_ok(N, ldc, out, residual, ldr, (col_scale, col_shift), *operands),
                         _x3_ok(C1, C2, N, hint if 0 < hint < M else M), _x3_resident(M, N, K, hint))
    if entry != "d3f_gemm_bf16" and (_h(A) or _h(skip) or _h(out)):
        raise TypeError("%s: bfloat16 operands that the bf16 contraction cannot address (K %d, lda %d)" % (what, K, lda))
    flags = [1 if leaky else 0, float(alpha)]
    if entry == "d3f_gemm_f32":
        ws = workspace(lib.d3f_gemm_workspace_bytes(M, N, K, hint), dev)
        args = [A.data_ptr(), lda, W.data_ptr(), ldb, out.data_ptr(), ldc, M, N, K, _ptr(row_scale), _ptr(col_scale), _ptr(col_shift),
                _ptr(residual), ldr] + flags + [ws.data_ptr(), ws.numel(), m_dev, hint]
    else:
        head = [A.data_ptr(), N1, lda, C1, _ptr(idx), ld_idx, _ptr(skip), lds, C2]
        if entry == "d3f_gemm_upsample_cat_f32":
            ws = workspace(lib.d3f_gemm_workspace_bytes(M, N, K, hint), dev)
            args = head + [W.data_ptr(), ldb, out.data_ptr(), ldc, M, N, _ptr(col_scale), _ptr(col_shift)] + flags
        else:
            pack, ws_bytes = {"d3f_gemm_bf16": (packed_bf16_weights, lib.d3f_gemm_bf16_workspace_bytes),
                              "d3f_gemm_f32t": (packed_f32t_weights, lib.d3f_gemm_workspace_bytes),
                              "d3f_gemm_x3": (packed_x3_weights, lib.d3f_gemm_x3_workspace_bytes)}[entry]
            Wp = pack(W)
            ws = workspace(ws_bytes(M, N, K, hint), dev)
            args = head + [Wp.data_ptr(), out.data_ptr(), ldc, M, N, _ptr(row_scale), _ptr(col_scale), _ptr(col_shift), _ptr(residual),
                           ldr] + flags
        args += [ws.data_ptr(), ws.numel(), m_dev, n1_dev, hint]
    if entry == "d3f_gemm_bf16":
        if out.data_ptr() % 16 or (residual is not None and (residual.data_ptr() % 8 or ldr % 4)):
            raise ValueError("gemm (bf16): output / residual must be 16 / 8-byte aligned with a leading dimension of 4 k")
        args += [_h(A), _h(out)]
    with _timed(name, dict(M=M, N=N, K=K), dev):
        rc = getattr(lib, entry)(*args, _stream(dev))
    _lib.check(rc, entry[4:])


def gemm(A, Bm, row_scale=None, col_scale=None, col_shift=None, residual=None, leaky=False, alpha=0.2, out=None):
    A, lda = _rows(_feat(A, "A"), "A")
    Bm, ldb = _rows(_req(Bm, torch.float32, "B"), "B")
    M, K = A.shape
    if Bm.shape[0] != K:
        raise ValueError("gemm: A is %s, B is %s" % (tuple(A.shape), tuple(Bm.shape)))
    N = Bm.shape[1]
    if out is None:
        out = torch.empty((M, N), dtype=_out_dtype(), device=A.device)
    out, ldc = _rows(out, "out")
    ldr = 0
    if residual is not None:
        residual, ldr = _rows(_feat(residual, "residual"), "residual")
    if (_h(A) or _h(out) or _h(residual)) and not (BF16_CONTRACTION and (residual is None or _h(residual) == _h(A))):
        raise TypeError("gemm: bfloat16 feature tensors need ops.bf16_contraction(features=True)")
    for v, n, name in ((row_scale, M, "row_scale"), (col_scale, N, "col_scale"), (col_shift, N, "col_shift")):
        if v is not None:
            _req(v, torch.float32, name)
            if v.numel() != n or not v.is_contiguous():
                raise ValueError("%s must be a contiguous vector of %d" % (name, n))
    _contract("gemm", A, M, lda, K, None, 0, None, 0, 0, Bm, ldb, out, ldc, _nd(A), None, int(getattr(A, "n_hint", 0) or 0),
              row_scale, col_scale, col_shift, residual, ldr, leaky, alpha)
    return _tag(out, A)


class UpsampleCat:

    def __init__(self, x, inds, skip=None):
        self.x, self.inds, self.skip = x, inds, skip
        self.shape = (inds.shape[0], x.shape[1] + (skip.shape[1] if skip is not None else 0))
        self.device = x.device
        _tag(self, inds)

    def materialize(self):
        return closest_pool_cat(self.x, self.inds, self.skip)


def gemm_upsample_cat(u, W, col_scale=None, col_shift=None, leaky=False, alpha=0.2):
    x, ldx = _rows(_feat(u.x, "x"), "x")
    inds, ldi = _rows(_req(u.inds, torch.int32, "inds"), "inds")
    W, ldb = _rows(_req(W, torch.float32, "W"), "W")
    C1, C2, lds, skip = x.shape[1], 0, 0, None
    if u.skip is not None:
        skip, lds = _rows(_feat(u.skip, "skip"), "skip")
        C2 = skip.shape[1]
    M, N = inds.shape[0], W.shape[1]
    if W.shape[0] != C1 + C2:
        raise ValueError("gemm_upsample_cat: W has %d rows, operands %d + %d columns" % (W.shape[0], C1, C2))
    if C2 and (C1 % 4 or lds % 4 or skip.data_ptr() % 16) and not _h(x):
        return gemm(u.materialize(), W, col_scale=col_scale, col_shift=col_shift, leaky=leaky, alpha=alpha)
    out = torch.empty((M, N), dtype=_out_dtype(), device=x.device)
    _contract("gemm_upsample_cat", x, x.shape[0], ldx, C1, inds, ldi, skip, lds, C2, W, ldb, out, N, _nd(inds), _nd(x),
              int(getattr(inds, "n_hint", 0) or 0), col_scale=col_scale, col_shift=col_shift, leaky=leaky, alpha=alpha)
    return _tag(out, inds)


DECODER_SPLIT = os.environ.get("D3F_DECODER_SPLIT", "1") != "0"


def _split_ok(M, C1, C2, N, hint=0, f32=True, f32t_ok=True):
    if not DECODER_SPLIT or BF16_CONTRACTION or not f32 or C2 <= 0 or C1 <= 0 or C1 % 32 or C2 % 32:
        return False
    resident = _x3_resident(M, N, C1 + C2, hint)
    entry, _ = _route(M, False, False, False, f32t_ok, _x3_ok(C1, C2, N, hint if 0 < hint < M else M), resident)
    return entry == "d3f_gemm_x3" and not resident


def upsample_split_ok(u, N):
    if u.skip is None or u.x.dim() != 2 or u.skip.dim() != 2 or u.inds.dim() != 2:
        return False
    f32 = u.x.dtype == torch.float32 and u.skip.dtype == torch.float32
    aligned = all(t.stride(1) == 1 and t.stride(0) % 4 == 0 and t.data_ptr() % 16 == 0 for t in (u.x, u.skip))
    return _split_ok(u.inds.shape[0], u.x.shape[1], u.skip.shape[1], N, int(getattr(u.inds, "n_hint", 0) or 0), f32, aligned and N % 4 == 0)


def gemm_upsample_split(u, W1, W2, col_shift=None, leaky=False, alpha=0.2, out=None):
    lib = _lib.load()
    x, _ = _rows(_req(u.x, torch.float32, "x"), "x")
    inds, ldi = _rows(_req(u.inds, torch.int32, "inds"), "inds")
    if u.skip is None:
        raise ValueError("gemm_upsample_split: no skip operand (use gemm_upsample_cat)")
    skip, lds = _rows(_req(u.skip, torch.float32, "skip"), "skip")
    W1, _ = _rows(_req(W1, torch.float32, "W1"), "W1")
    W2, _ = _rows(_req(W2, torch.float32, "W2"), "W2")
    C1, C2, M, N = x.shape[1], skip.shape[1], inds.shape[0], W2.shape[1]
    if W1.shape != (C1, N) or W2.shape[0] != C2 or skip.shape[0] != M or not (W1.is_contiguous() and W2.is_contiguous()):
        raise ValueError("gemm_upsample_split: operands %s | %s, W1 %s, W2 %s" % (tuple(x.shape), tuple(skip.shape), tuple(W1.shape),
                                                                                   tuple(W2.shape)))
    if not upsample_split_ok(u, N):
        raise ValueError("gemm_upsample_split: not a call of the split form (ops.upsample_split_ok): use gemm_upsample_cat")
    Y = gemm(x, W1)
    dev, hint = x.device, int(getattr(inds, "n_hint", 0) or 0)
    if out is None:
        out = torch.empty((M, N), dtype=torch.float32, device=dev)
    elif out.dtype != torch.float32 or tuple(out.shape) != (M, N) or not out.is_contiguous() or out.data_ptr() % 16:
        raise ValueError("gemm_upsample_split: out must be a contiguous, 16-byte aligned float32 [%d, %d]" % (M, N))
    if col_shift is not None and (col_shift.data_ptr() % 16 or col_shift.numel() != N):
        raise ValueError("gemm_upsample_split: col_shift must be a 16-byte aligned vector of %d" % N)
    Wp = packed_x3_weights(W2)
    ws = workspace(lib.d3f_gemm_x3_workspace_bytes(M, N, C2, hint), dev)
    with _timed("gemm_x3", dict(M=M, N=N, K=C2), dev):
        rc = lib.d3f_gemm_x3_gres(skip.data_ptr(), M, lds, C2, None, 0, None, 0, 0, Wp.data_ptr(), out.data_ptr(), N, M, N, None, None,
                                  _ptr(col_shift), Y.data_ptr(), N, inds.data_ptr(), ldi, x.shape[0], _nd(x), 1 if leaky else 0,
                                  float(alpha), ws.data_ptr(), ws.numel(), _nd(inds), None, hint, _stream(dev))
    _lib.check(rc, "gemm_x3_gres")
    return _tag(out, inds)


def gemm_cat2(A1, A2, W, col_scale=None, col_shift=None, leaky=False, alpha=0.2):
    A1, ld1 = _rows(_feat(A1, "A1"), "A1")
    A2, ld2 = _rows(_feat(A2, "A2"), "A2")
    W, ldb = _rows(_req(W, torch.float32, "W"), "W")
    M, C1, C2, N = A1.shape[0], A1.shape[1], A2.shape[1], W.shape[1]
    if A2.shape[0] != M or W.shape[0] != C1 + C2:
        raise ValueError("gemm_cat2: operands %s | %s, W %s" % (tuple(A1.shape), tuple(A2.shape), tuple(W.shape)))
    if (C1 % 4 or ld2 % 4 or A2.data_ptr() % 16) and not _h(A1):
        return gemm(torch.cat([A1, A2], 1), W, col_scale=col_scale, col_shift=col_shift, leaky=leaky, alpha=alpha)
    out = torch.empty((M, N), dtype=_out_dtype(), device=A1.device)
    _contract("gemm_cat2", A1, M, ld1, C1, None, 0, A2, ld2, C2, W, ldb, out, N, _nd(A1), _nd(A1), int(getattr(A1, "n_hint", 0) or 0),
              col_scale=col_scale, col_shift=col_shift, leaky=leaky, alpha=alpha)
    return _tag(out, A1)


def _kp_front(what, query_points, support_points, neighbors_indices, features, K_points, K_values, KP_extent, KP_influence,
              aggregation_mode, col_scale=None, col_shift=None, residual=None, leaky=False, alpha=0.2, row_pos=True, feat=_feat):
    lib = _lib.load()
    q = _req(query_points, torch.float32, "query_points", 2).contiguous()
    s = _req(support_points, torch.float32, "support_points", 2).contiguous()
    idx, ld_idx = _rows(_req(neighbors_indices, torch.int32, "neighbors_indices"), "neighbors_indices")
    f, ldf = _rows(feat(features, "features"), "features")
    if KP_influence not in _INFLUENCE:
        raise ValueError("Unknown influence function type (config.KP_influence)")
    if aggregation_mode not in _AGGREGATION:
        raise ValueError("Unknown convolution mode. Should be 'closest' or 'sum'")
    if K_values is not None and f.shape[1] != K_values.shape[1]:
        raise ValueError("%s: features have %d channels, K_values expects %d" % (what, f.shape[1], K_values.shape[1]))
    kp = _kp_host(K_points)
    Nq, Ns = q.shape[0], s.shape[0]
    nq_dev, ns_dev = _nd(query_points), _nd(support_points)
    if ns_dev is None:
        ns_dev = _nd(features)
    rpos = None
    if row_pos:
        rpos = torch.empty((max(Ns, 1),), dtype=torch.uint8, device=q.device)
        _lib.check(lib.d3f_row_positive(f.data_ptr(), Ns, ldf, f.shape[1], rpos.data_ptr(), ns_dev, _h(f), _stream(q.device)),
                   "row_positive")
    ldr = 0
    if residual is not None:
        residual, ldr = _rows(_req(residual, torch.float32, "residual"), "residual")
    return ((q, Nq, s, Ns, idx, ld_idx, idx.shape[1], f, ldf),
            (kp, kp.shape[0], float(KP_extent), _INFLUENCE[KP_influence], _AGGREGATION[aggregation_mode]), rpos,
            (col_scale, col_shift, residual, ldr, 1 if leaky else 0, float(alpha)), (nq_dev, ns_dev, _order(query_points)), f)


def _arg(v):
    if isinstance(v, torch.Tensor):
        return v.data_ptr()
    return v.ctypes.data if isinstance(v, np.ndarray) else v


def kpconv_aggregate(query_points, support_points, neighbors_indices, features, K_points, KP_extent,
                     KP_influence="linear", aggregation_mode="sum"):
    lib = _lib.load()
    if neighbors_indices.shape[0] != query_points.shape[0] or features.shape[0] != support_points.shape[0]:
        raise ValueError("KPConv: %d queries / %d index rows, %d supports / %d feature rows" %
                         (query_points.shape[0], neighbors_indices.shape[0], support_points.shape[0], features.shape[0]))
    gather, kpar, row_pos, _, tail, f = _kp_front("KPConv", query_points, support_points, neighbors_indices, features, K_points, None,
                                                  KP_extent, KP_influence, aggregation_mode)
    Nq, Ns, K, Cin = gather[1], gather[3], gather[6], f.shape[1]
    wf = torch.empty((Nq, kpar[1] * Cin), dtype=torch.float32, device=f.device)
    inv_cnt = torch.empty((Nq,), dtype=torch.float32, device=f.device)
    with _timed("kpconv_aggregate", dict(Nq=Nq, Ns=Ns, K=K, Cin=Cin), f.device):
        rc = lib.d3f_kpconv_aggregate(*map(_arg, (*gather, Cin, row_pos, *kpar, wf, inv_cnt, *tail, _h(f), _stream(f.device))))
    _lib.check(rc, "kpconv_aggregate")
    return _tag(wf, query_points), _tag(inv_cnt, query_points)


def kpconv_deform_aggregate(query_points, support_points, neighbors_indices, features, K_points, offsets, KP_extent,
                            KP_influence="linear", aggregation_mode="sum", modulations=None, raw=False):
    lib = _lib.load()
    if neighbors_indices.shape[0] != query_points.shape[0] or features.shape[0] != support_points.shape[0]:
        raise ValueError("KPConv_deformable: %d queries / %d index rows, %d supports / %d feature rows" %
                         (query_points.shape[0], neighbors_indices.shape[0], support_points.shape[0], features.shape[0]))
    if isinstance(features, torch.Tensor) and features.dtype == torch.bfloat16:
        raise TypeError("KPConv_deformable reads float32 feature rows only: d3f_kpconv_deform_aggregate has no bfloat16 "
                        "feature-storage form")
    gather, kpar, _, _, tail, f = _kp_front("KPConv_deformable", query_points, support_points, neighbors_indices, features, K_points,
                                            None, KP_extent, KP_influence, aggregation_mode, row_pos=False,
                                            feat=lambda t, name: _req(t, torch.float32, name))
    Nq, Ns, K, Cin, num_kp = gather[1], gather[3], gather[6], f.shape[1], kpar[1]
    _req(offsets, torch.float32, "offsets")
    if offsets.dim() == 3:
        offsets = offsets.reshape(offsets.shape[0], -1)
    off, ld_off = _rows(offsets, "offsets")
    mod, ld_mod = None, 0
    if raw:
        if modulations is not None or tuple(off.shape) not in ((Nq, 3 * num_kp), (Nq, 4 * num_kp)):
            raise ValueError("KPConv_deformable: raw offsets are %s, expected (%d, %d) or (%d, %d) and no modulations"
                             % (tuple(off.shape), Nq, 3 * num_kp, Nq, 4 * num_kp))
        if off.shape[1] == 4 * num_kp:
            mod, ld_mod = off[:, 3 * num_kp:], ld_off
    else:
        if tuple(off.shape) != (Nq, 3 * num_kp):
            raise ValueError("KPConv_deformable: offsets are %s, expected (%d, %d, 3)" % (tuple(offsets.shape), Nq, num_kp))
        if modulations is not None:
            mod, ld_mod = _rows(_req(modulations, torch.float32, "modulations"), "modulations")
            if tuple(mod.shape) != (Nq, num_kp):
                raise ValueError("KPConv_deformable: modulations are %s, expected (%d, %d)" % (tuple(mod.shape), Nq, num_kp))
    wf = torch.empty((Nq, num_kp * Cin), dtype=torch.float32, device=f.device)
    with _timed("kpconv_deform_aggregate", dict(Nq=Nq, Ns=Ns, K=K, Cin=Cin), f.device):
        rc = lib.d3f_kpconv_deform_aggregate(*map(_arg, (*gather, Cin, off, ld_off, float(KP_extent) if raw else 1.0, mod, ld_mod,
                                                         1 if raw else 0, *kpar, wf, *tail, 0, _stream(f.device))))
    _lib.check(rc, "kpconv_deform_aggregate")
    return _tag(wf, query_points)


def kpconv_deformable(query_points, support_points, neighbors_indices, features, K_points, K_values, offset_weights, offset_bias,
                      KP_extent, KP_influence="linear", aggregation_mode="sum", modulated=False, col_scale=None, col_shift=None,
                      residual=None, leaky=False, alpha=0.2):
    num_kp, cin, cout = K_values.shape
    D = (4 if modulated else 3) * num_kp
    if tuple(offset_weights.shape) != (num_kp, cin, D) or tuple(offset_bias.shape) != (D,):
        raise ValueError("KPConv_deformable: offset_conv_weights %s / offset_conv_bias %s, expected (%d, %d, %d) / (%d,)" %
                         (tuple(offset_weights.shape), tuple(offset_bias.shape), num_kp, cin, D, D))
    if features.shape[1] != cin:
        raise ValueError("KPConv_deformable: features have %d channels, K_values expects %d" % (features.shape[1], cin))
    with f32_output():
        wf0, inv_cnt = kpconv_aggregate(query_points, support_points, neighbors_indices, features, K_points, KP_extent, KP_influence,
                                        aggregation_mode)
        offsets = gemm(wf0, offset_weights.reshape(num_kp * cin, D), row_scale=inv_cnt, col_shift=offset_bias)
    wf = kpconv_deform_aggregate(query_points, support_points, neighbors_indices, features, K_points, offsets, KP_extent,
                                 KP_influence, aggregation_mode, raw=True)
    return gemm(wf, K_values.reshape(num_kp * cin, cout), col_scale=col_scale, col_shift=col_shift, residual=residual, leaky=leaky,
                alpha=alpha)


def kpconv_fused_supported(cin, cout, num_kp, KP_influence, aggregation_mode, available=False):
    r = _lib.load().d3f_kpconv_fused_supported(int(cin), int(cout), int(num_kp), _INFLUENCE.get(KP_influence, -1),
                                               _AGGREGATION.get(aggregation_mode, -1))
    return r >= 1 if available else r == 1


def _packed_kpconv(K_values, slot, alloc, pack, what):
    def make(t):
        num_kp, cin, cout = K_values.shape
        W = _req(K_values, torch.float32, "K_values").reshape(num_kp * cin, cout).contiguous()
        if t is None:
            t = alloc(W)
        _lib.check(pack(W.data_ptr(), num_kp * cin, cout, t.data_ptr(), _stream(W.device)), what)
        return t
    return _packed_on_tensor(K_values, slot, make)


def packed_kpconv_weights(K_values):
    return _packed_kpconv(K_values, "_d3f_packed", torch.empty_like, _lib.load().d3f_kpconv_pack_weights, "kpconv_pack_weights")


def packed_kpconv_weights_x3(K_values):
    lib = _lib.load()
    return _packed_kpconv(K_values, "_d3f_packed_x3",
                          lambda W: torch.empty((int(lib.d3f_kpconv_packed_x3_bytes(*W.shape)) // 2,), dtype=torch.int16, device=W.device),
                          lib.d3f_kpconv_pack_weights_x3, "kpconv_pack_weights_x3")


_PACKERS = (("_d3f_bf16t", packed_bf16_weights), ("_d3f_f32t", packed_f32t_weights), ("_d3f_x3", packed_x3_weights),
            ("_d3f_packed", packed_kpconv_weights), ("_d3f_packed_x3", packed_kpconv_weights_x3))


KP_X3 = os.environ.get("D3F_KP_X3", "1") != "0"


def _kpconv_fused(what, query_points, support_points, neighbors_indices, features, K_points, K_values, KP_extent, KP_influence,
                  aggregation_mode, col_scale, col_shift, residual, leaky, alpha):
    lib = _lib.load()
    num_kp, cin, cout = K_values.shape
    gather, kpar, row_pos, epi, tail, f = _kp_front(what, query_points, support_points, neighbors_indices, features, K_points, K_values,
                                                    KP_extent, KP_influence, aggregation_mode, col_scale, col_shift, residual, leaky,
                                                    alpha)
    level0 = what == "kpconv_fused32"
    x3 = KP_X3 and (num_kp * cin) % 32 == 0 and (level0 or cout % 16 == 0)
    if x3:
        W = packed_kpconv_weights_x3(K_values)
    elif level0:
        W = _req(K_values, torch.float32, "K_values").reshape(num_kp * cin, cout).contiguous()
    else:
        W = packed_kpconv_weights(K_values)
    out = torch.empty((gather[1], cout), dtype=f.dtype, device=f.device)
    with _timed(what, dict(Nq=gather[1], Ns=gather[3], K=gather[6], Cin=cin, Cout=cout), f.device):
        if level0:
            rc = (lib.d3f_kpconv_fused32_x3 if x3 else lib.d3f_kpconv_fused32)(
                *map(_arg, (*gather, row_pos, *kpar, W, *epi, out, cout, *tail, _h(f), _stream(f.device))))
        else:
            rc = (lib.d3f_kpconv_fused_x3 if x3 else lib.d3f_kpconv_fused)(
                *map(_arg, (*gather, cin, row_pos, *kpar, W, cout, *epi, out, cout, *tail, _h(f), _stream(f.device))))
    _lib.check(rc, what)
    return _tag(out, query_points)


def kpconv_fused32(query_points, support_points, neighbors_indices, features, K_points, K_values, KP_extent,
                   KP_influence="linear", aggregation_mode="sum", col_scale=None, col_shift=None, residual=None,
                   leaky=False, alpha=0.2):
    if tuple(K_values.shape[1:]) != (32, 32):
        raise ValueError("kpconv_fused32 needs Cin == Cout == 32")
    return _kpconv_fused("kpconv_fused32", query_points, support_points, neighbors_indices, features, K_points, K_values, KP_extent,
                         KP_influence, aggregation_mode, col_scale, col_shift, residual, leaky, alpha)


def kpconv_fused(query_points, support_points, neighbors_indices, features, K_points, K_values, KP_extent,
                 KP_influence="linear", aggregation_mode="sum", col_scale=None, col_shift=None, residual=None,
                 leaky=False, alpha=0.2):
    return _kpconv_fused("kpconv_fused", query_points, support_points, neighbors_indices, features, K_points, K_values, KP_extent,
                         KP_influence, aggregation_mode, col_scale, col_shift, residual, leaky, alpha)


def kpconv_fused_c1(query_points, support_points, neighbors_indices, features, K_points, K_values, KP_extent,
                    KP_influence="linear", aggregation_mode="sum", col_scale=None, col_shift=None, residual=None,
                    leaky=False, alpha=0.2):
    lib = _lib.load()
    num_kp, cin, cout = K_values.shape
    if cin != 1:
        raise ValueError("kpconv_fused_c1 needs Cin == 1")
    gather, kpar, _, epi, tail, f = _kp_front("kpconv_fused_c1", query_points, support_points, neighbors_indices, features, K_points,
                                              K_values, KP_extent, KP_influence, aggregation_mode, col_scale, col_shift, residual,
                                              leaky, alpha, row_pos=False, feat=lambda t, name: _req(t, torch.float32, name))
    W = _req(K_values, torch.float32, "K_values").reshape(num_kp, cout).contiguous()
    out = torch.empty((gather[1], cout), dtype=torch.bfloat16 if BF16_FEATURES else torch.float32, device=f.device)
    with _timed("kpconv_fused_c1", dict(Nq=gather[1], Ns=gather[3], K=gather[6], Cin=1, Cout=cout), f.device):
        rc = lib.d3f_kpconv_fused_c1(*map(_arg, (*gather, *kpar, W, cout, *epi, out, cout, *tail, _h(out), _stream(f.device))))
    _lib.check(rc, "kpconv_fused_c1")
    return _tag(out, query_points)


def ind_max_pool(x, inds):
    lib = _lib.load()
    x, ldx = _rows(_feat(x, "x"), "x")
    inds, ldi = _rows(_req(inds, torch.int32, "inds"), "inds")
    dev = x.device
    out = torch.empty((inds.shape[0], x.shape[1]), dtype=x.dtype, device=dev)
    with _timed("ind_max_pool", dict(N1=x.shape[0], N2=inds.shape[0], K=inds.shape[1], C=x.shape[1]), dev):
        rc = lib.d3f_ind_max_pool(x.data_ptr(), x.shape[0], ldx, x.shape[1], inds.data_ptr(), inds.shape[0], ldi,
                                  inds.shape[1], out.data_ptr(), x.shape[1], None, _nd(x), _nd(inds), _order(inds),
                                  _h(x), _stream(dev))
    _lib.check(rc, "ind_max_pool")
    return _tag(out, inds)


def closest_pool_cat(x, inds, skip=None):
    lib = _lib.load()
    x, ldx = _rows(_req(x, torch.float32, "x"), "x")
    inds, ldi = _rows(_req(inds, torch.int32, "inds"), "inds")
    dev = x.device
    C1 = x.shape[1]
    C2 = lds = 0
    if skip is not None:
        skip, lds = _rows(_req(skip, torch.float32, "skip"), "skip")
        C2 = skip.shape[1]
        if skip.shape[0] != inds.shape[0]:
            raise ValueError("closest_pool_cat: %d index rows, %d skip rows" % (inds.shape[0], skip.shape[0]))
    out = torch.empty((inds.shape[0], C1 + C2), dtype=torch.float32, device=dev)
    rc = lib.d3f_closest_pool_cat(x.data_ptr(), x.shape[0], ldx, C1, inds.data_ptr(), inds.shape[0], ldi,
                                  _ptr(skip), lds, C2, out.data_ptr(), C1 + C2,
                                  _nd(x), _nd(inds), _stream(dev))
    _lib.check(rc, "closest_pool_cat")
    return _tag(out, inds)


def detect_head(x, neighbors, stack_lengths_dev, include_zero_dev, stack_group=0):
    lib = _lib.load()
    x, ldx = _rows(_req(x, torch.float32, "x"), "x")
    nb, ldi = _rows(_req(neighbors, torch.int32, "neighbors"), "neighbors")
    dev = x.device
    N, Cc = x.shape
    B = stack_lengths_dev.numel()
    desc = torch.empty((N, Cc), dtype=torch.float32, device=dev)
    score = torch.empty((N, 1), dtype=torch.float32, device=dev)
    scratch = torch.empty((2 * B + 2 + (N + 3) // 4,), dtype=torch.int32, device=dev)
    with _timed("detect_head", dict(N=N, K=nb.shape[1], C=Cc), dev):
        rc = lib.d3f_detect_head(x.data_ptr(), N, ldx, Cc, nb.data_ptr(), ldi, nb.shape[1],
                                 stack_lengths_dev.data_ptr(),
                                 _ptr(include_zero_dev),
                                 int(stack_group), B, desc.data_ptr(), Cc, score.data_ptr(), scratch.data_ptr(), _order(nb),
                                 _stream(dev))
    _lib.check(rc, "detect_head")
    return _tag(desc, x), _tag(score, x)


def _typed(t, dtype, name, ndim=None):
    if not isinstance(t, torch.Tensor):
        raise TypeError("%s must be a torch.Tensor on a GPU (got %s)" % (name, type(t)))
    if t.dtype != dtype:
        raise TypeError("%s must be %s (got %s)" % (name, dtype, t.dtype))
    if ndim is not None and t.dim() != ndim:
        raise ValueError("%s must be %d-D (got shape %s)" % (name, ndim, tuple(t.shape)))
    return t


def _head_arguments(what, x, neighbors, stack_lengths_dev):
    nb, ldi = _rows(_typed(neighbors, torch.int32, "neighbors"), "neighbors")
    lens = _typed(stack_lengths_dev, torch.int32, "stack_lengths_dev", 1)
    if not lens.is_contiguous():
        raise ValueError("%s: stack_lengths_dev must be contiguous" % what)
    if not 1 <= lens.numel() <= 255:
        raise ValueError("%s: %d clouds (1 .. 255)" % (what, lens.numel()))
    if nb.shape[0] * nb.shape[1] > (1 << 31) - 8192:
        raise ValueError("%s: %d x %d neighbour slots (at most 2^31 - 8192)" % (what, nb.shape[0], nb.shape[1]))
    if x is not None and x.shape[0] != nb.shape[0]:
        raise ValueError("%s: %d feature rows, %d neighbour rows" % (what, x.shape[0], nb.shape[0]))
    return nb, ldi, lens


def _on_device(what, **tensors):
    for name, t in tensors.items():
        if t is not None and not t.is_cuda:
            raise _lib.D3FeatLibraryError("%s: %s is on %s: d3feat_amd has no CPU path" % (what, name, t.device))


def neighbor_transpose(neighbors, stack_lengths_dev):
    lib = _lib.load()
    nb, ldi, lens = _head_arguments("neighbor_transpose", None, neighbors, stack_lengths_dev)
    _on_device("neighbor_transpose", neighbors=nb, stack_lengths_dev=lens)
    dev = nb.device
    N, K = nb.shape
    start = torch.empty((N + 1,), dtype=torch.int32, device=dev)
    edges = torch.empty((max(N * K, 1),), dtype=torch.int32, device=dev)
    nbytes = lib.d3f_neighbor_transpose_workspace_bytes(N, K)
    ws = workspace(nbytes, dev)
    with _timed("neighbor_transpose", dict(N=N, K=K), dev):
        rc = lib.d3f_neighbor_transpose(nb.data_ptr(), N, ldi, K, lens.data_ptr(), lens.numel(), start.data_ptr(), edges.data_ptr(),
                                        ws.data_ptr(), nbytes, _stream(dev))
    _lib.check(rc, "neighbor_transpose")
    return start, edges[:N * K]


def detect_head_backward(x, neighbors, stack_lengths_dev, include_zero_dev, grad_desc, grad_score, stack_group=0, transpose=None,
                         out=None):
    lib = _lib.load()
    x, ldx = _rows(_typed(x, torch.float32, "x"), "x")
    nb, ldi, lens = _head_arguments("detect_head_backward", x, neighbors, stack_lengths_dev)
    dev = x.device
    N, Cc = x.shape
    if not 1 <= Cc <= 128:
        raise ValueError("detect_head_backward: C = %d (1 .. 128)" % Cc)
    if int(stack_group) < 0:
        raise ValueError("detect_head_backward: stack_group = %r" % (stack_group,))
    gd = ldg = gs = ldgs = None
    if grad_desc is not None:
# ... 121 lines not shown
```

### include/d3feat_amd.h

```cpp
#ifndef D3FEAT_AMD_H
#define D3FEAT_AMD_H

#include <stddef.h>
#include <stdint.h>

#ifdef __cplusplus
extern "C" {
#endif

#define D3F_OK 0
#define D3F_ERR_HIP (-1)
#define D3F_ERR_WORKSPACE (-2)
#define D3F_ERR_ARG (-3)

#define D3F_ST_EMPTY_ELEMENT 1
#define D3F_ST_NEG_CELL 2
#define D3F_ST_KEY_RANGE 4
#define D3F_ST_HIT_OVERFLOW 8
#define D3F_ST_OUT_OVERFLOW 16
#define D3F_ST_KEY_WIDTH 32

#define D3F_NB_NO_KMAX 2
#define D3F_PAD_NUM_SUPPORTS (-2147483647 - 1)

#define D3F_MAX_BATCH 255
#define D3F_NEIGHBOR_CAP 1024
#define D3F_TOPK_MAX 8192
#define D3F_PAIRS_KMAX 1024
#define D3F_REPEAT_COUNTS_MAX 16
#define D3F_SCENES_MAX 256
#define D3F_MATCH_KMAX 8192
#define D3F_VALIDATION_NMAX 1024
#define D3F_NUM_KP_MAX 16

int d3f_version(void);

int d3f_trace_marker(int id, void* stream);
int d3f_pack_status(int* dst, const int* a, int na, const int* b, int nb, const int* c, int nc, const int* d, int nd,
                    int* clear, int nclear, int clear_first, int clear_step, void* stream);


size_t d3f_grid_subsample_workspace_bytes(int N, int B, int fdim, int ldim);
int d3f_batch_grid_subsample_async(const float* points, int N_cap, const int* lens_dev, int B, float dl,
                                   float* sub_points, int M_cap, int elem_cap, int elem_points_cap, int* sub_lens_dev,
                                   int* status_dev, void* workspace, size_t workspace_bytes, void* stream);
int d3f_batch_grid_subsample_async_inplace(const float* const* clouds_dev, int N_cap, const int* lens_dev, int B, float dl,
                                           float* sub_points, int M_cap, int elem_cap, int* sub_lens_dev, int* status_dev,
                                           void* workspace, size_t workspace_bytes, void* stream);

int d3f_stack_self_pair(const float* pts, int M_cap, const int* lens_in_dev, int B, float* out, int* lens_out_dev,
                        int* total_dev, void* stream);
int d3f_stack_self_pair_boxed(const float* pts, int M_cap, const int* lens_in_dev, int B, float* out, int* lens_out_dev,
                              int* total_dev, const unsigned* bbox_in_dev, unsigned* bbox_out_dev, void* stream);
int d3f_batch_grid_subsample_async_boxed(const float* points, const float* const* clouds_dev, int N_cap, const int* lens_dev,
                                         int B, float dl, float* sub_points, int M_cap, int elem_cap, int elem_points_cap,
                                         int* sub_lens_dev, int* status_dev, const unsigned* bbox_in_dev,
                                         unsigned* bbox_out_dev, void* workspace, size_t workspace_bytes, void* stream);
int d3f_batch_grid_subsample(const float* points, int N, const int* lens_dev, int B, float dl,
                             const float* features, int fdim, const int* classes, int ldim,
                             float* sub_points, float* sub_features, int* sub_classes, int* sub_lens_dev,
                             int* status_host, void* workspace, size_t workspace_bytes, void* stream);

size_t d3f_radius_neighbors_workspace_bytes(int Nq, int Ns, int B);
int d3f_batch_radius_neighbors(const float* queries, int Nq, const float* supports, int Ns,
                               const int* q_lens_dev, const int* s_lens_dev, int B, float radius,
                               int* out, int ld, int width, int pad_value, int* status_dev,
                               void* workspace, size_t workspace_bytes, void* stream);

size_t d3f_neighbor_grid_bytes(int Ns, int B);
size_t d3f_neighbor_grid_order_offset(int Ns, int B);
int d3f_neighbor_grid_build(const float* supports, int Ns, const int* s_lens_dev, int B, float radius,
                            void* grid, size_t grid_bytes, void* stream);
#define D3F_GRID_RESET_MAX 8
int d3f_neighbor_grid_boxed_form(int Ns, int B);
int d3f_geometry_reset(unsigned* boxes_dev, int n_boxes, const void* const* grids, const size_t* grid_bytes, const int* Ns,
                       const int* B, int n_grids, void* stream);
int d3f_neighbor_grid_build_boxed(const float* supports, int Ns, const int* s_lens_dev, int B, float radius,
                                  const unsigned* bbox_dev, void* grid, size_t grid_bytes, void* stream);
int d3f_neighbor_grid_search(const void* grid, size_t grid_bytes, int Ns, const float* queries, int Nq,
                             const int* q_lens_dev, int B, float radius, int queries_are_supports,
                             int* out, int ld, int width, int pad_value, int cap, int first_only, float nn_hint,
                             int reset_status, int* status_dev, void* stream);
#define D3F_NB_INTERNAL 4
int d3f_neighbor_grid_search_ordered(const void* grid, size_t grid_bytes, int Ns, const float* queries, int Nq,
                                     const int* q_lens_dev, int B, float radius, const void* query_grid, size_t query_grid_bytes,
                                     int* out, int ld, int width, int pad_value, int cap, int first_only, float nn_hint, int flags,
                                     int* status_dev, void* stream);
size_t d3f_neighbor_grid_inv_offset(int Ns, int B);
size_t d3f_neighbor_grid_xyz_offset(int Ns, int B);



int d3f_row_positive(const void* f, int Ns, int ldf, int Cin, unsigned char* row_pos, const int* Ns_dev, int feat_bf16,
                     void* stream);
int d3f_kpconv_aggregate(const float* q, int Nq, const float* s, int Ns, const int* idx, int ld_idx, int K,
                         const void* f, int ldf, int Cin, const unsigned char* row_pos, const float* kp_host,
                         int num_kp, float KP_extent, int influence, int aggregation, float* wf, float* inv_cnt,
                         const int* Nq_dev, const int* Ns_dev, const int* q_order, int feat_bf16, void* stream);

int d3f_kpconv_deform_aggregate(const float* q, int Nq, const float* s, int Ns, const int* idx, int ld_idx, int K,
                                const void* f, int ldf, int Cin, const float* offsets, int ld_off, float offset_scale,
                                const float* modulations, int ld_mod, int mod_logits, const float* kp_host, int num_kp,
                                float KP_extent, int influence, int aggregation, float* wf, const int* Nq_dev, const int* Ns_dev,
                                const int* q_order, int feat_bf16, void* stream);

int d3f_kpconv_fused_c1(const float* q, int Nq, const float* s, int Ns, const int* idx, int ld_idx, int K,
                        const float* f, int ldf, const float* kp_host, int num_kp, float KP_extent, int influence,
                        int aggregation, const float* W, int Cout, const float* col_scale, const float* col_shift,
                        const float* residual, int ldr, int leaky, float alpha, void* out, int ldo,
                        const int* Nq_dev, const int* Ns_dev, const int* q_order, int out_bf16, void* stream);

int d3f_kpconv_fused32(const float* q, int Nq, const float* s, int Ns, const int* idx, int ld_idx, int K,
                       const void* f, int ldf, const unsigned char* row_pos, const float* kp_host, int num_kp,
                       float KP_extent, int influence, int aggregation, const float* W, const float* col_scale,
                       const float* col_shift, const float* residual, int ldr, int leaky, float alpha, void* out, int ldo,
                       const int* Nq_dev, const int* Ns_dev, const int* q_order, int feat_bf16, void* stream);

int d3f_kpconv_fused_supported(int Cin, int Cout, int num_kp, int influence, int aggregation);
int d3f_kpconv_pack_weights(const float* W, int K, int N, float* W_packed, void* stream);
size_t d3f_kpconv_packed_x3_bytes(int K, int N);
int d3f_kpconv_pack_weights_x3(const float* W, int K, int N, void* W_planes, void* stream);
int d3f_kpconv_fused32_x3(const float* q, int Nq, const float* s, int Ns, const int* idx, int ld_idx, int K,
                          const void* f, int ldf, const unsigned char* rowpos, const float* kp_host, int num_kp,
                          float KP_extent, int influence, int aggregation, const float* W_planes, const float* col_scale,
                          const float* col_shift, const float* residual, int ldr, int leaky, float alpha, void* out,
                          int ldo, const int* Nq_dev, const int* Ns_dev, const int* q_order, int feat_bf16, void* stream);
int d3f_kpconv_fused_x3(const float* q, int Nq, const float* s, int Ns, const int* idx, int ld_idx, int K,
                        const void* f, int ldf, int Cin, const unsigned char* rowpos, const float* kp_host, int num_kp,
                        float KP_extent, int influence, int aggregation, const float* W_planes, int Cout,
                        const float* col_scale, const float* col_shift, const float* residual, int ldr, int leaky,
                        float alpha, void* out, int ldo, const int* Nq_dev, const int* Ns_dev, const int* q_order,
                        int feat_bf16, void* stream);
int d3f_kpconv_fused(const float* q, int Nq, const float* s, int Ns, const int* idx, int ld_idx, int K,
                     const void* f, int ldf, int Cin, const unsigned char* rowpos, const float* kp_host, int num_kp,
                     float KP_extent, int influence, int aggregation, const float* W_packed, int Cout,
                     const float* col_scale, const float* col_shift, const float* residual, int ldr, int leaky,
                     float alpha, void* out, int ldo, const int* Nq_dev, const int* Ns_dev, const int* q_order,
                     int feat_bf16, void* stream);

size_t d3f_gemm_workspace_bytes(int M, int N, int K, int M_hint);
int d3f_gemm_f32(const float* A, int lda, const float* B, int ldb, float* C, int ldc, int M, int N, int K,
                 const float* row_scale, const float* col_scale, const float* col_shift,
                 const float* residual, int ldr, int leaky, float alpha,
                 void* workspace, size_t workspace_bytes, const int* M_dev, int M_hint, void* stream);

int d3f_gemm_upsample_cat_f32(const float* x, int N1, int ldx, int C1, const int* idx, int ld_idx,
                              const float* skip, int lds, int C2, const float* W, int ldb, float* C, int ldc,
                              int M, int N, const float* col_scale, const float* col_shift, int leaky, float alpha,
                              void* workspace, size_t workspace_bytes, const int* M_dev, const int* N1_dev,
                              int M_hint, void* stream);

int d3f_ind_max_pool(const void* x, int N1, int ldx, int C, const int* idx, int N2, int ld_idx, int K,
                     void* out, int ldo, float* col_min_dev, const int* N1_dev, const int* N2_dev, const int* row_order,
                     int feat_bf16, void* stream);
int d3f_closest_pool_cat(const float* x, int N1, int ldx, int C1, const int* idx, int N2, int ld_idx,
                         const float* skip, int lds, int C2, float* out, int ldo, const int* N1_dev, const int* N2_dev,
                         void* stream);

int d3f_affine_act(const float* x, int ldx, int M, int N, const float* col_scale, const float* col_shift,
                   const float* residual, int ldr, int leaky, float alpha, float* out, int ldo, const int* M_dev,
                   void* stream);

int d3f_detect_head(const float* x, int N, int ldx, int C, const int* idx, int ld_idx, int K,
                    const int* lens_dev, const int* include_zero_dev, int stack_group, int B, float* desc, int ldd,
                    float* score, int* scratch_dev, const int* row_order, void* stream);

int d3f_pack_descriptors(const float* xyz, const float* desc, int ldd, int C, const float* score, int N, float* out,
                         int ldo, const int* N_dev, void* stream);
int d3f_pack_descriptors_to(const float* xyz, const float* desc, int ldd, int C, const float* score, int N, float* out,
                            int ldo, const int* N_dev, const int* lens_dev, int B, int group, int keep,
                            const long long* dst_ptrs_dev, const int* row_map_dev, void* stream);

size_t d3f_topk_workspace_bytes(int N, int B, int n_cap, int K);
int d3f_topk_records(const float* xyz, int ldx, const float* desc, int ldd, int C, const float* score, int lds, int N,
                     const int* N_dev, const int* lens_dev, int B, int group, int keep, const int* row_map_dev, int n_cap, int K,
                     float* out, int ldo, int* idx_out, int* count_dev, int* tickets_dev, void* workspace, size_t workspace_bytes,
                     void* stream);

int d3f_gemm_pack_f32t(const float* W, int ldb, int K, int N, float* Wt, void* stream);
int d3f_gemm_f32t(const float* A, int N1, int lda, int C1, const int* idx, int ld_idx, const float* skip, int lds, int C2,
                  const float* Wt, float* C, int ldc, int M, int N, const float* row_scale, const float* col_scale,
                  const float* col_shift, const float* residual, int ldr, int leaky, float alpha, void* workspace,
                  size_t workspace_bytes, const int* M_dev, const int* N1_dev, int M_hint, void* stream);

size_t d3f_gemm_x3_packed_bytes(int K, int N);
int d3f_gemm_pack_x3(const float* W, int ldb, int K, int N, void* Wx, void* stream);
size_t d3f_gemm_x3_workspace_bytes(int M, int N, int K, int M_hint);
int d3f_gemm_x3_plan(int M, int N, int K, int M_hint, int* rows, int* cols, int* slices);
int d3f_gemm_x3_resident(int M, int N, int K, int M_hint);
int d3f_gemm_x3(const float* A, int N1, int lda, int C1, const int* idx, int ld_idx, const float* skip, int lds, int C2,
                const void* Wx, float* C, int ldc, int M, int N, const float* row_scale, const float* col_scale,
                const float* col_shift, const float* residual, int ldr, int leaky, float alpha, void* workspace,
                size_t workspace_bytes, const int* M_dev, const int* N1_dev, int M_hint, void* stream);
int d3f_gemm_x3_gres(const float* A, int N1, int lda, int C1, const int* idx, int ld_idx, const float* skip, int lds, int C2,
                     const void* Wx, float* C, int ldc, int M, int N, const float* row_scale, const float* col_scale,
                     const float* col_shift, const float* residual, int ldr, const int* res_idx, int ld_res_idx, int res_rows,
                     const int* res_rows_dev, int leaky, float alpha, void* workspace, size_t workspace_bytes, const int* M_dev,
                     const int* N1_dev, int M_hint, void* stream);

size_t d3f_gemm_bf16_workspace_bytes(int M, int N, int K, int M_hint);
int d3f_gemm_pack_bf16(const float* W, int ldb, int K, int N, void* W_packed, void* stream);
int d3f_gemm_bf16(const void* A, int N1, int lda, int C1, const int* idx, int ld_idx, const void* skip, int lds, int C2,
                  const void* W_packed, void* C, int ldc, int M, int N, const float* row_scale, const float* col_scale,
                  const float* col_shift, const void* residual, int ldr, int leaky, float alpha, void* workspace,
                  size_t workspace_bytes, const int* M_dev, const int* N1_dev, int M_hint, int a_bf16, int c_bf16, void* stream);

int d3f_decode_xyz_records(const void* raw, int n, int stride, int off_x, int off_y, int off_z, int is_f64, int big_endian,
                           float* out, void* stream);


size_t d3f_feature_nn_workspace_bytes(int Na);
int d3f_feature_nn(const float* A, int Na, int lda, const float* B, int Nb, int ldb, int C, int* idx, float* d2_out,
                   void* workspace, size_t workspace_bytes, void* stream);

size_t d3f_mutual_matches_workspace_bytes(int Na);
int d3f_mutual_matches(const int* ab, int Na, const int* ba, int Nb, int* pairs, int* count_dev, void* workspace,
                       size_t workspace_bytes, void* stream);

int d3f_ransac_hypotheses(const float* src, int Ns, const float* tgt, int Nt, const int* nn, int ransac_n,
                          float edge_similarity, float checker_distance, uint64_t seed, uint64_t it0,
                          int H, float* T_out, unsigned char* valid_out, void* stream);
int d3f_ransac_draw(uint64_t seed, uint64_t iteration, int d, int n);

int d3f_neighbor_grid_score(const void* grid, size_t grid_bytes, int Nt, const float* src, int Ns, const float* T, int V,
                            float radius, int* count_dev, uint64_t* sumd2_dev, int* nearest_dev, void* stream);

size_t d3f_register_pairs_workspace_bytes(int P, int K, int num_keypts, int max_validation);
int d3f_register_pairs(const float* kp, int n_blocks, int K, int ld, int C, const int* count_dev, const int* pairs_dev, int P,
                       int num_keypts, float max_correspondence_distance, int ransac_n, float edge_similarity,
                       float checker_distance, int max_iteration, int max_validation, uint64_t seed, const float* gt,
                       float distance_threshold, float* T_out, int* inliers, uint64_t* sumd2, int* validations, int* iterations,
                       int* best_iteration, int* mutual_count, int* nearest, int* mutual, int* gt_inliers, void* workspace,
                       size_t workspace_bytes, void* stream);

int d3f_repeatability_pairs(const float* kp, int n_blocks, int K, int ld, const int* count_dev, const int* pairs_dev, int P,
                            const double* gt_dev, int moved, const double* threshold_host, const int* num_keypts_host,
                            int n_counts, int* repeat_dev, int64_t* totals_dev, void* stream);

size_t d3f_match_pairs_workspace_bytes(int P, const int* num_keypts_host, int n_counts);
int d3f_match_pairs(const float* kp, int n_blocks, int K, int ld, int C, const int* count_dev, const int* pairs_dev, int P,
                    const float* gt, float distance_threshold, const int* num_keypts_host, int n_counts, int* mutual_count,
                    int* gt_inliers, void* workspace, size_t workspace_bytes, void* stream);

size_t d3f_register_pairs_counts_workspace_bytes(int P, int n_blocks, int K, const int* num_keypts_host, int n_counts,
                                                 int max_validation);
int d3f_register_pairs_counts(const float* kp, int n_blocks, int K, int ld, int C, const int* count_dev, const int* pairs_dev, int P,
                              const int* num_keypts_host, int n_counts, float max_correspondence_distance, int ransac_n,
                              float edge_similarity, float checker_distance, int max_iteration, int max_validation, uint64_t seed,
                              const float* gt, float distance_threshold, float* T_out, int* inliers, uint64_t* sumd2,
                              int* validations, int* iterations, int* best_iteration, int* mutual_count, int* gt_inliers,
                              int* nearest, void* workspace, size_t workspace_bytes, void* stream);

int d3f_overlap_pairs(const void* grid, size_t grid_bytes, int N, int B, const int* pairs_dev, int P, float threshold,
                      int* count_dev, int* nearest_dev, int ld_nearest, void* stream);

size_t d3f_validation_pairs_workspace_bytes(int P, int ld_idx);
int d3f_validation_pairs(const float* desc, int ldd, int C, const float* score, int lds, const float* points, int ldp, int n_rows,
                         const int* row0_dev, const int* anc_dev, const int* pos_dev, int ld_idx, const int* n_dev, int P,
                         float safe_radius, int keypts_num, float det_loss_weight, float pos_margin, float neg_margin,
                         float log_scale, float* values, int* status_dev, double* sums_dev, int64_t* counts_dev, void* workspace,
                         size_t workspace_bytes, void* stream);

size_t d3f_loss_gradients_workspace_bytes(int P, int ld_idx, int C);
int d3f_loss_gradients(const float* desc, int ldd, int C, const float* score, int lds, const float* points, int ldp, int n_rows,
                       const int* row0_dev, const int* anc_dev, const int* pos_dev, int ld_idx, const int* n_dev, int P,
                       float safe_radius, int keypts_num, float det_loss_weight, float pos_margin, float neg_margin, float log_scale,
                       int contrastive, float* grad_desc, int ldg, float* grad_score, int ldgs, float* values, int* status_dev,
                       void* workspace, size_t workspace_bytes, void* stream);

size_t d3f_neighbor_transpose_workspace_bytes(int N, int K);
int d3f_neighbor_transpose(const int* idx, int N, int ld_idx, int K, const int* lens_dev, int B, int* start, int* edges, void* workspace,
                           size_t workspace_bytes, void* stream);

size_t d3f_detect_head_backward_workspace_bytes(int N, int C, int B);
int d3f_detect_head_backward(const float* x, int N, int ldx, int C, const int* idx, int ld_idx, int K, const int* lens_dev,
                             const int* include_zero_dev, int stack_group, int B, const int* start, const int* edges,
                             const float* gdesc, int ldg, const float* gscore, int ldgs, float* gx, int ldgx, void* workspace,
                             size_t workspace_bytes, void* stream);

int d3f_pose_errors(const float* T_est, const float* gt, int P, int per_pair, const double* thresholds_host, double* rte_dev,
                    double* rre_deg_dev, int* flags_dev, double* meters_dev, void* stream);

int d3f_sanitize_descriptors(float* kp, int n_blocks, int K, int ld, int C, void* stream);

int d3f_matching_summary(const int* mutual_count, const int* gt_inliers, const int* gt_flag, int P, int n, const int* scene_start_host,
                         int S, const double* inlier_ratio_host, int* ratio_e8, long long* figures, void* stream);

int d3f_registration_recall(const void* T_est, int logged, const double* gt, const double* info, const int* gt_flag,
                            const int* result_flag, const int* ids, int P, int n, const int* scene_start_host, int S,
                            const double* err2_host, double* error, int* flags, long long* figures, void* stream);

size_t d3f_icp_pairs_workspace_bytes(int N_src, int B);
int d3f_icp_pairs(const void* grid, size_t grid_bytes, int N_tgt, const float* src, int N_src, const int* src_lens_dev, int B,
                  const double* init, const double* criteria_host, int max_iteration, int check_every, double* T, int* count,
                  double* sumd2, double* fitness, double* rmse, int* iterations, int* converged, int* nearest, void* workspace,
                  size_t workspace_bytes, void* stream);

#ifdef __cplusplus
}
#endif
#endif
```

Before: 1941 fragments/s.

## Fuse row-positive flag computation into the unary GEMM epilogue

The conv1 unary GEMM in ResNet blocks now computes per-row positive-sum flags inside its epilogue (resident, tiled, and split-K reduce paths) and tags the output tensor with them. The later KPConv aggregation reuses these flags instead of launching a separate row_positive kernel that re-reads the feature matrix. This removes one kernel launch and one full read of the activations per block. In exchange the GEMM epilogue does extra double-precision accumulation and a cross-lane shuffle, and a small uint8 buffer is allocated per call. Version-based tag checks guard against stale reuse.

```diff
diff --git a/d3feat_amd/_lib.py b/d3feat_amd/_lib.py
--- a/d3feat_amd/_lib.py
+++ b/d3feat_amd/_lib.py
@@ -122,6 +122,10 @@
                          _vp, _vp, _i, _vp]),
     "d3f_gemm_x3_gres": (_i, [_vp, _i, _i, _i, _vp, _i, _vp, _i, _i, _vp, _vp, _i, _i, _i, _vp, _vp, _vp, _vp, _i, _vp, _i, _i, _vp, _i, _f,
                               _vp, _sz, _vp, _vp, _i, _vp]),
+    "d3f_gemm_x3_rowpos": (_i, [_vp, _i, _i, _i, _vp, _i, _vp, _i, _i, _vp, _vp, _i, _i, _i, _vp, _vp, _vp, _vp, _i, _i, _f, _vp, _sz,
+                                _vp, _vp, _i, _vp, _vp]),
+    "d3f_gemm_x3_gres_rowpos": (_i, [_vp, _i, _i, _i, _vp, _i, _vp, _i, _i, _vp, _vp, _i, _i, _i, _vp, _vp, _vp, _vp, _i, _vp, _i, _i, _vp,
+                                     _i, _f, _vp, _sz, _vp, _vp, _i, _vp, _vp]),
     "d3f_gemm_bf16": (_i, [_vp, _i, _i, _i, _vp, _i, _vp, _i, _i, _vp, _vp, _i, _i, _i, _vp, _vp, _vp, _vp, _i, _i, _f, _vp, _sz,
                            _vp, _vp, _i, _i, _i, _vp]),
     "d3f_decode_xyz_records": (_i, [_vp, _i, _i, _i, _i, _i, _i, _i, _vp, _vp]),
diff --git a/d3feat_amd/csrc/gemm_common.h b/d3feat_amd/csrc/gemm_common.h
--- a/d3feat_amd/csrc/gemm_common.h
+++ b/d3feat_amd/csrc/gemm_common.h
@@ -28,7 +28,10 @@
     int ld_ridx;
     int res_rows;
     const int* res_rows_dev;
+    unsigned char* rowpos;
 };
+
+__device__ __forceinline__ double gemm_row_sum_halves(double s) { return s + __shfl_xor(s, 32, 64); }
 
 __device__ __forceinline__ const float* gemm_residual_row(const GemmEpi& E, int m) {
     if (!E.ridx) return E.residual + (size_t)m * E.ldr;
@@ -65,12 +68,8 @@
     }
 }
 
-__global__ void __launch_bounds__(256)
-gemm_splitk_reduce_kernel(const float* __restrict__ slab, int S, int M, int N, float* __restrict__ C, int ldc, GemmEpi E,
-                          const int* __restrict__ M_dev, int res_bf16 = 0, int c_bf16 = 0) {
-    const long long i = (long long)blockIdx.x * blockDim.x + threadIdx.x;
-    if (i >= (long long)d3f_dyn(M, M_dev) * N) return;
-    const int m = (int)(i / N), n = (int)(i % N);
+__device__ __forceinline__ float gemm_splitk_value(const float* __restrict__ slab, int S, int M, int N, float* __restrict__ C, int ldc,
+                                                   GemmEpi E, int m, int n, int res_bf16, int c_bf16) {
     float v = 0.f;
     for (int s = 0; s < S; ++s) v += slab[((size_t)s * M + m) * N + n];
     if (res_bf16 && E.residual) {
@@ -92,6 +91,35 @@
     }
     if (c_bf16) ((unsigned short*)C)[(size_t)m * ldc + n] = (unsigned short)d3f_bf16_rne(v);
     else C[(size_t)m * ldc + n] = v;
+    return v;
+}
+
+__global__ void __launch_bounds__(256)
+gemm_splitk_reduce_kernel(const float* __restrict__ slab, int S, int M, int N, float* __restrict__ C, int ldc, GemmEpi E,
+                          const int* __restrict__ M_dev, int res_bf16 = 0, int c_bf16 = 0) {
+    const long long i = (long long)blockIdx.x * blockDim.x + threadIdx.x;
+    if (i >= (long long)d3f_dyn(M, M_dev) * N) return;
+    gemm_splitk_value(slab, S, M, N, C, ldc, E, (int)(i / N), (int)(i % N), res_bf16, c_bf16);
+}
+
+__global__ void __launch_bounds__(256)
+gemm_splitk_reduce_rowpos_kernel(const float* __restrict__ slab, int S, int M, int N, float* __restrict__ C, int ldc, GemmEpi E,
+                                 const int* __restrict__ M_dev) {
+    __shared__ double part[4];
+    const long long i = (long long)blockIdx.x * blockDim.x + threadIdx.x;
+    const bool in = i < (long long)d3f_dyn(M, M_dev) * N;
+    double s = in ? (double)gemm_splitk_value(slab, S, M, N, C, ldc, E, (int)(i / N), (int)(i % N), 0, 0) : 0.0;
+#pragma unroll
+    for (int o = 32; o > 0; o >>= 1)
+        if (o < N) s += __shfl_xor(s, o, 64);
+    if (N > 64) {
+        const int w = threadIdx.x >> 6, per = N >> 6;
+        if ((threadIdx.x & 63) == 0) part[w] = s;
+        __syncthreads();
+        s = 0.0;
+        for (int k = 0; k < per; ++k) s += part[(w & ~(per - 1)) + k];
+    }
+    if (in && i % N == 0) E.rowpos[i / N] = s > 0.0 ? 1 : 0;
 }
 
 static inline size_t gemm_slab_bytes(int S, int M, int N) { return S > 1 ? d3f_align((size_t)S * M * N * sizeof(float)) + 256 : 256; }
@@ -107,7 +135,9 @@
 
 static inline void gemm_reduce(const float* slab, int S, int M, int N, float* C, int ldc, const GemmEpi& E, const int* M_dev,
                                hipStream_t stream, int res_bf16 = 0, int c_bf16 = 0) {
-    if (S > 1)
+    if (S > 1 && E.rowpos && !res_bf16 && !c_bf16 && N <= 256 && (N & (N - 1)) == 0)
+        gemm_splitk_reduce_rowpos_kernel<<<d3f_cdiv((long long)M * N, 256), 256, 0, stream>>>(slab, S, M, N, C, ldc, E, M_dev);
+    else if (S > 1)
         gemm_splitk_reduce_kernel<<<d3f_cdiv((long long)M * N, 256), 256, 0, stream>>>(slab, S, M, N, C, ldc, E, M_dev, res_bf16, c_bf16);
 }
 
diff --git a/d3feat_amd/csrc/gemm_f32.hip b/d3feat_amd/csrc/gemm_f32.hip
--- a/d3feat_amd/csrc/gemm_f32.hip
+++ b/d3feat_amd/csrc/gemm_f32.hip
@@ -707,17 +707,21 @@
                        const void* Wx, float* C, int ldc, int M, int N, const float* row_scale, const float* col_scale,
                        const float* col_shift, const float* residual, int ldr, const int* res_idx, int ld_res_idx, int res_rows,
                        const int* res_rows_dev, int leaky, float alpha, void* workspace, size_t workspace_bytes, const int* M_dev,
-                       const int* N1_dev, int M_hint, void* stream_) {
+                       const int* N1_dev, int M_hint, void* stream_, unsigned char* rowpos = nullptr, int* rowpos_written = nullptr) {
     hipStream_t stream = (hipStream_t)stream_;
     const int K = C1 + C2;
+    if (rowpos_written) *rowpos_written = 0;
     bool empty;
     if (int rc = gemm_check_composite(true, GX_BK, 15, M, N, N1, C1, C2, lda, ldc, lds, ldr, ld_idx, A, Wx, C, idx, skip, residual,
                                       col_scale, col_shift, empty))
         return rc;
     if (res_idx && (ld_res_idx < 1 || res_rows < 0)) return D3F_ERR_ARG;
-    if (empty) return D3F_OK;
+    if (empty) {
+        if (rowpos && rowpos_written) *rowpos_written = 1;
+        return D3F_OK;
+    }
     if (res_idx && !residual) return D3F_ERR_ARG;
-    GemmEpi E{row_scale, col_scale, col_shift, residual, ldr, leaky, alpha, res_idx, ld_res_idx, res_rows, res_rows_dev};
+    GemmEpi E{row_scale, col_scale, col_shift, residual, ldr, leaky, alpha, res_idx, ld_res_idx, res_rows, res_rows_dev, nullptr};
     GemmGather G{idx, ld_idx, N1, N1_dev, C2 > 0 ? skip : nullptr, lds, C1};
     const int nkt = K / GX_BK, NG = d3f_cdiv(N, 32);
     if (!res_idx && d3f_gemm_x3_resident(M, N, K, M_hint)) {
@@ -735,10 +739,20 @@
         const void* const fns[3] = {(const void*)gemm_x3r_kernel<1>, (const void*)gemm_x3r_kernel<2>, (const void*)gemm_x3r_kernel<4>};
         if (d3f_opt_in_lds(lds_done, fns, 160 * 1024) != D3F_OK) return D3F_ERR_HIP;
         const int grid = std::min(cus, d3f_cdiv(d3f_cdiv(M, 32), 8));
-#define D3F_GXR(TN_) gemm_x3r_kernel<TN_><<<grid, 512, gemm_x3r_lds_bytes(nkt, NG), stream>>>(A, lda, (const unsigned short*)Wx, nkt, C, ldc, M, N, E, M_dev, G)
-        if (NG == 4) D3F_GXR(4);
-        else if (NG == 2) D3F_GXR(2);
-        else D3F_GXR(1);
+        E.rowpos = rowpos;
+        if (rowpos && rowpos_written) *rowpos_written = 1;
+#define D3F_GXR(K_, TN_) K_<TN_><<<grid, 512, gemm_x3r_lds_bytes(nkt, NG), stream>>>(A, lda, (const unsigned short*)Wx, nkt, C, ldc, M, N, E, M_dev, G)
+        if (rowpos) {
+            static std::atomic<unsigned long long> lds_done_rp{0};
+            const void* const fns_rp[3] = {(const void*)gemm_x3r_rowpos_kernel<1>, (const void*)gemm_x3r_rowpos_kernel<2>,
+                                           (const void*)gemm_x3r_rowpos_kernel<4>};
+            if (d3f_opt_in_lds(lds_done_rp, fns_rp, 160 * 1024) != D3F_OK) return D3F_ERR_HIP;
+            if (NG == 4) D3F_GXR(gemm_x3r_rowpos_kernel, 4);
+            else if (NG == 2) D3F_GXR(gemm_x3r_rowpos_kernel, 2);
+            else D3F_GXR(gemm_x3r_rowpos_kernel, 1);
+        } else if (NG == 4) D3F_GXR(gemm_x3r_kernel, 4);
+        else if (NG == 2) D3F_GXR(gemm_x3r_kernel, 2);
+        else D3F_GXR(gemm_x3r_kernel, 1);
 #undef D3F_GXR
         D3F_LAUNCH_CHECK();
         return D3F_OK;
@@ -749,10 +763,18 @@
     if (int rc = gemm_slab(S, M, N, workspace, workspace_bytes, slab)) return rc;
     if (d3f_cdiv(M, bm) > 65535) return D3F_ERR_ARG;
     dim3 grid(d3f_cdiv(N, 32 * pl.tn), S, d3f_cdiv(M, bm));
-#define D3F_GX(TN_, WV_) gemm_x3_kernel<TN_, WV_><<<grid, 64 * WV_, 0, stream>>>(A, lda, (const unsigned short*)Wx, nkt, NG, C, ldc, M, N, tps, slab, E, M_dev, G)
-    if (pl.waves == 8) D3F_GX(4, 8);
-    else if (pl.tn == 1) D3F_GX(1, 4);
-    else D3F_GX(2, 4);
+    if (rowpos && N <= 128 && (S > 1 ? (N & (N - 1)) == 0 : grid.x == 1)) {
+        E.rowpos = rowpos;
+        if (rowpos_written) *rowpos_written = 1;
+    }
+#define D3F_GX(K_, TN_, WV_) K_<TN_, WV_><<<grid, 64 * WV_, 0, stream>>>(A, lda, (const unsigned short*)Wx, nkt, NG, C, ldc, M, N, tps, slab, E, M_dev, G)
+    if (E.rowpos && S == 1) {
+        if (pl.waves == 8) D3F_GX(gemm_x3_rowpos_kernel, 4, 8);
+        else if (pl.tn == 1) D3F_GX(gemm_x3_rowpos_kernel, 1, 4);
+        else D3F_GX(gemm_x3_rowpos_kernel, 2, 4);
+    } else if (pl.waves == 8) D3F_GX(gemm_x3_kernel, 4, 8);
+    else if (pl.tn == 1) D3F_GX(gemm_x3_kernel, 1, 4);
+    else D3F_GX(gemm_x3_kernel, 2, 4);
 #undef D3F_GX
     gemm_reduce(slab, S, M, N, C, ldc, E, M_dev, stream);
     D3F_LAUNCH_CHECK();
@@ -776,3 +798,26 @@
                        res_idx, ld_res_idx, res_rows, res_rows_dev, leaky, alpha, workspace, workspace_bytes, M_dev, N1_dev, M_hint,
                        stream_);
 }
+
+extern "C" int d3f_gemm_x3_gres_rowpos(const float* A, int N1, int lda, int C1, const int* idx, int ld_idx, const float* skip, int lds,
+                                       int C2, const void* Wx, float* C, int ldc, int M, int N, const float* row_scale,
+                                       const float* col_scale, const float* col_shift, const float* residual, int ldr,
+                                       const int* res_idx, int ld_res_idx, int res_rows, const int* res_rows_dev, int leaky, float alpha,
+                                       void* workspace, size_t workspace_bytes, const int* M_dev, const int* N1_dev, int M_hint,
+                                       unsigned char* row_pos, void* stream_) {
+    int written = 0;
+    const int rc = gemm_x3_run(A, N1, lda, C1, idx, ld_idx, skip, lds, C2, Wx, C, ldc, M, N, row_scale, col_scale, col_shift, residual,
+                               ldr, res_idx, ld_res_idx, res_rows, res_rows_dev, leaky, alpha, workspace, workspace_bytes, M_dev, N1_dev,
+                               M_hint, stream_, row_pos, &written);
+    return rc != D3F_OK ? rc : written;
+}
+
+extern "C" int d3f_gemm_x3_rowpos(const float* A, int N1, int lda, int C1, const int* idx, int ld_idx, const float* skip, int lds, int C2,
+                                  const void* Wx, float* C, int ldc, int M, int N, const float* row_scale, const float* col_scale,
+                                  const float* col_shift, const float* residual, int ldr, int leaky, float alpha, void* workspace,
+                                  size_t workspace_bytes, const int* M_dev, const int* N1_dev, int M_hint, unsigned char* row_pos,
+                                  void* stream_) {
+    return d3f_gemm_x3_gres_rowpos(A, N1, lda, C1, idx, ld_idx, skip, lds, C2, Wx, C, ldc, M, N, row_scale, col_scale, col_shift,
+                                   residual, ldr, nullptr, 0, 0, nullptr, leaky, alpha, workspace, workspace_bytes, M_dev, N1_dev, M_hint,
+                                   row_pos, stream_);
+}
diff --git a/d3feat_amd/csrc/gemm_x3.h b/d3feat_amd/csrc/gemm_x3.h
--- a/d3feat_amd/csrc/gemm_x3.h
+++ b/d3feat_amd/csrc/gemm_x3.h
@@ -78,11 +78,10 @@
     else static_assert(NB < 0, "add the round");
 }
 
-template <int TN, int WAVES>
-__global__ void __launch_bounds__(64 * WAVES) __attribute__((amdgpu_waves_per_eu(2, 2)))
-gemm_x3_kernel(const float* __restrict__ A, int lda, const unsigned short* __restrict__ Wx, int nkt, int NG, float* __restrict__ C,
-               int ldc, int M, int N, int tiles_per_split, float* __restrict__ slab, GemmEpi E, const int* __restrict__ M_dev,
-               GemmGather G) {
+template <int TN, int WAVES, bool RP>
+__device__ __forceinline__ void gemm_x3_body(const float* __restrict__ A, int lda, const unsigned short* __restrict__ Wx, int nkt, int NG,
+                                             float* __restrict__ C, int ldc, int M, int N, int tiles_per_split, float* __restrict__ slab,
+                                             GemmEpi E, const int* __restrict__ M_dev, GemmGather G) {
     constexpr int BM = 32 * WAVES, BN = 32 * TN, NTH = 64 * WAVES;
     constexpr int NB = (480 * TN + NTH - 1) / NTH;
     constexpr int SB = NB * NTH * 16;
@@ -254,6 +253,8 @@
     const float* rrow = (!slab && E.residual && mok) ? gemm_residual_row(E, gm_a) : nullptr;
     static_assert(3 * SB >= WAVES * 32 * 36 * 4, "the output patches must fit the ring");
     float* patch = (float*)Bs + wave * (32 * 36);
+    const bool flags = RP && !slab && E.rowpos && gridDim.x == 1;
+    double rsum = 0.0;
 #pragma unroll
     for (int j = 0; j < TN; ++j) {
         if (!slab) {
@@ -272,6 +273,7 @@
                         t += rr[e];
                         v[e] = (E.leaky && !(t > 0.f)) ? t * E.alpha : t;
                     }
+                    if constexpr (RP) rsum += (double)v[0] + (double)v[1] + (double)v[2] + (double)v[3];
                 }
                 *(float4*)&patch[(lane & 31) * 36 + 8 * q + 4 * (lane >> 5)] = make_float4(v[0], v[1], v[2], v[3]);
             }
@@ -309,15 +311,37 @@
             *(float4*)&dst[gn] = make_float4(v[0], v[1], v[2], v[3]);
         }
     }
+    if constexpr (RP) {
+        if (flags) {
+            rsum = gemm_row_sum_halves(rsum);
+            if (mok && lane < 32) E.rowpos[gm_a] = rsum > 0.0 ? 1 : 0;
+        }
+    }
+}
+
+template <int TN, int WAVES>
+__global__ void __launch_bounds__(64 * WAVES) __attribute__((amdgpu_waves_per_eu(2, 2)))
+gemm_x3_kernel(const float* __restrict__ A, int lda, const unsigned short* __restrict__ Wx, int nkt, int NG, float* __restrict__ C,
+               int ldc, int M, int N, int tiles_per_split, float* __restrict__ slab, GemmEpi E, const int* __restrict__ M_dev,
+               GemmGather G) {
+    gemm_x3_body<TN, WAVES, false>(A, lda, Wx, nkt, NG, C, ldc, M, N, tiles_per_split, slab, E, M_dev, G);
+}
+
+template <int TN, int WAVES>
+__global__ void __launch_bounds__(64 * WAVES) __attribute__((amdgpu_waves_per_eu(2, 2)))
+gemm_x3_rowpos_kernel(const float* __restrict__ A, int lda, const unsigned short* __restrict__ Wx, int nkt, int NG, float* __restrict__ C,
+                      int ldc, int M, int N, int tiles_per_split, float* __restrict__ slab, GemmEpi E, const int* __restrict__ M_dev,
+                      GemmGather G) {
+    gemm_x3_body<TN, WAVES, true>(A, lda, Wx, nkt, NG, C, ldc, M, N, tiles_per_split, slab, E, M_dev, G);
 }
 
 #define GXR_PS 36
 #define GXR_PATCH_BYTES (8 * 32 * GXR_PS * 4)
 #define GXR_EPI_BYTES (2 * 128 * 4)
-template <int TN>
-__global__ void __launch_bounds__(512) __attribute__((amdgpu_waves_per_eu(2, 2)))
-gemm_x3r_kernel(const float* __restrict__ A, int lda, const unsigned short* __restrict__ Wx, int nkt, float* __restrict__ C, int ldc,
-                int M, int N, GemmEpi E, const int* __restrict__ M_dev, GemmGather G) {
+template <int TN, bool RP>
+__device__ __forceinline__ void gemm_x3r_body(const float* __restrict__ A, int lda, const unsigned short* __restrict__ Wx, int nkt,
+                                              float* __restrict__ C, int ldc, int M, int N, GemmEpi E,
+                                              const int* __restrict__ M_dev, GemmGather G) {
     extern __shared__ __attribute__((aligned(16))) unsigned char gxr_w[];
     static_assert(TN == 1 || TN == 2 || TN == 4, "column groups per row tile");
     M = d3f_dyn(M, M_dev);
@@ -451,6 +475,7 @@
         const bool mok = gm_a < M;
         float rs = 1.f;
         if (E.row_scale && mok) rs = E.row_scale[gm_a];
+        double rsum = 0.0;
 #pragma unroll
         for (int j = 0; j < TN; ++j) {
 #pragma unroll
@@ -468,6 +493,7 @@
                         tt += rr[e];
                         v[e] = (E.leaky && !(tt > 0.f)) ? tt * E.alpha : tt;
                     }
+                    if constexpr (RP) rsum += (double)v[0] + (double)v[1] + (double)v[2] + (double)v[3];
                 }
                 *(float4*)&patch[(lane & 31) * GXR_PS + 8 * q + 4 * (lane >> 5)] = make_float4(v[0], v[1], v[2], v[3]);
                 acc[j][4 * q] = acc[j][4 * q + 1] = acc[j][4 * q + 2] = acc[j][4 * q + 3] = 0.f;
@@ -484,6 +510,10 @@
             }
             __builtin_amdgcn_fence(__ATOMIC_ACQUIRE, "wavefront");
             __builtin_amdgcn_wave_barrier();
+        }
+        if constexpr (RP) {
+            rsum = gemm_row_sum_halves(rsum);
+            if (mok && lane < 32) E.rowpos[gm_a] = rsum > 0.0 ? 1 : 0;
         }
         c_tile += tstride;
     };
@@ -515,3 +545,17 @@
     asm volatile("s_waitcnt vmcnt(0)" : "+v"(rA0), "+v"(rA1), "+v"(rA2), "+v"(rA3), "+v"(rB0), "+v"(rB1), "+v"(rB2), "+v"(rB3), "+v"(rC0),
                  "+v"(rC1), "+v"(rC2), "+v"(rC3) : : "memory");
 }
+
+template <int TN>
+__global__ void __launch_bounds__(512) __attribute__((amdgpu_waves_per_eu(2, 2)))
+gemm_x3r_kernel(const float* __restrict__ A, int lda, const unsigned short* __restrict__ Wx, int nkt, float* __restrict__ C, int ldc,
+                int M, int N, GemmEpi E, const int* __restrict__ M_dev, GemmGather G) {
+    gemm_x3r_body<TN, false>(A, lda, Wx, nkt, C, ldc, M, N, E, M_dev, G);
+}
+
+template <int TN>
+__global__ void __launch_bounds__(512) __attribute__((amdgpu_waves_per_eu(2, 2)))
+gemm_x3r_rowpos_kernel(const float* __restrict__ A, int lda, const unsigned short* __restrict__ Wx, int nkt, float* __restrict__ C,
+                       int ldc, int M, int N, GemmEpi E, const int* __restrict__ M_dev, GemmGather G) {
+    gemm_x3r_body<TN, true>(A, lda, Wx, nkt, C, ldc, M, N, E, M_dev, G);
+}
diff --git a/d3feat_amd/kernels/convolution_ops.py b/d3feat_amd/kernels/convolution_ops.py
--- a/d3feat_amd/kernels/convolution_ops.py
+++ b/d3feat_amd/kernels/convolution_ops.py
@@ -6,8 +6,8 @@
 
 
 
-def unary_convolution(features, K_values, epilogue=None):
-    return ops.gemm(features, K_values, **(epilogue or {}))
+def unary_convolution(features, K_values, epilogue=None, row_pos=False):
+    return ops.gemm(features, K_values, row_pos=row_pos, **(epilogue or {}))
 
 
 def KPConv(query_points, support_points, neighbors_indices, features, K_values, fixed='center', KP_extent=1.0,
diff --git a/d3feat_amd/models/network_blocks.py b/d3feat_amd/models/network_blocks.py
--- a/d3feat_amd/models/network_blocks.py
+++ b/d3feat_amd/models/network_blocks.py
@@ -141,7 +141,7 @@
     cin = int(features.shape[1])
     with variable_scope('conv1'):
         w = weight_variable([cin, fdim // 2])
-        x = conv_ops.unary_convolution(features, w, epilogue=_epilogue(fdim // 2, config, True))
+        x = conv_ops.unary_convolution(features, w, epilogue=_epilogue(fdim // 2, config, True), row_pos=not deformable)
     with variable_scope('conv2'):
         w = weight_variable([config.num_kernel_points, fdim // 2, fdim // 2])
         if strided:
diff --git a/d3feat_amd/ops.py b/d3feat_amd/ops.py
--- a/d3feat_amd/ops.py
+++ b/d3feat_amd/ops.py
@@ -584,8 +584,17 @@
     return True
 
 
+ROWPOS_EPI = os.environ.get("D3F_ROWPOS_EPI", "1") != "0"
+
+
+def _tag_row_pos(out, flags):
+    if flags is not None:
+        out.row_pos = (flags, out._version)
+    return out
+
+
 def _contract(what, A, N1, lda, C1, idx, ld_idx, skip, lds, C2, W, ldb, out, ldc, m_dev, n1_dev, hint, row_scale=None, col_scale=None,
-              col_shift=None, residual=None, ldr=0, leaky=False, alpha=0.2):
+              col_shift=None, residual=None, ldr=0, leaky=False, alpha=0.2, row_pos=False):
     lib = _lib.load()
     (M, N), K, dev = out.shape, C1 + C2, out.device
     operands = ((A, lda, C1), (skip, lds, C2))
@@ -618,12 +627,19 @@
         if out.data_ptr() % 16 or (residual is not None and (residual.data_ptr() % 8 or ldr % 4)):
             raise ValueError("gemm (bf16): output / residual must be 16 / 8-byte aligned with a leading dimension of 4 k")
         args += [_h(A), _h(out)]
+    rpos = None
+    if row_pos and ROWPOS_EPI and entry == "d3f_gemm_x3":
+        entry, rpos = "d3f_gemm_x3_rowpos", torch.empty((max(M, 1),), dtype=torch.uint8, device=dev)
+        args.append(rpos.data_ptr())
     with _timed(name, dict(M=M, N=N, K=K), dev):
         rc = getattr(lib, entry)(*args, _stream(dev))
+    if rpos is not None and rc in (0, 1):
+        rc, rpos = _lib.D3F_OK, (rpos if rc == 1 else None)
     _lib.check(rc, entry[4:])
-
-
-def gemm(A, Bm, row_scale=None, col_scale=None, col_shift=None, residual=None, leaky=False, alpha=0.2, out=None):
+    return rpos
+
+
+def gemm(A, Bm, row_scale=None, col_scale=None, col_shift=None, residual=None, leaky=False, alpha=0.2, out=None, row_pos=False):
     A, lda = _rows(_feat(A, "A"), "A")
     Bm, ldb = _rows(_req(Bm, torch.float32, "B"), "B")
     M, K = A.shape
@@ -643,9 +659,9 @@
             _req(v, torch.float32, name)
             if v.numel() != n or not v.is_contiguous():
                 raise ValueError("%s must be a contiguous vector of %d" % (name, n))
-    _contract("gemm", A, M, lda, K, None, 0, None, 0, 0, Bm, ldb, out, ldc, _nd(A), None, int(getattr(A, "n_hint", 0) or 0),
-              row_scale, col_scale, col_shift, residual, ldr, leaky, alpha)
-    return _tag(out, A)
+    flags = _contract("gemm", A, M, lda, K, None, 0, None, 0, 0, Bm, ldb, out, ldc, _nd(A), None, int(getattr(A, "n_hint", 0) or 0),
+                      row_scale, col_scale, col_shift, residual, ldr, leaky, alpha, row_pos)
+    return _tag_row_pos(_tag(out, A), flags)
 
 
 class UpsampleCat:
@@ -766,6 +782,11 @@
         ns_dev = _nd(features)
     rpos = None
     if row_pos:
+        have = getattr(features, "row_pos", None)
+        if ROWPOS_EPI and have is not None and f is features and have[1] == f._version and have[0].numel() >= max(Ns, 1) and \
+                f.shape[0] == Ns and (ns_dev is not None or _nd(features) is None):
+            rpos = have[0]
+    if row_pos and rpos is None:
         rpos = torch.empty((max(Ns, 1),), dtype=torch.uint8, device=q.device)
         _lib.check(lib.d3f_row_positive(f.data_ptr(), Ns, ldf, f.shape[1], rpos.data_ptr(), ns_dev, _h(f), _stream(q.device)),
                    "row_positive")
diff --git a/include/d3feat_amd.h b/include/d3feat_amd.h
--- a/include/d3feat_amd.h
+++ b/include/d3feat_amd.h
@@ -197,6 +197,15 @@
                      const float* col_shift, const float* residual, int ldr, const int* res_idx, int ld_res_idx, int res_rows,
                      const int* res_rows_dev, int leaky, float alpha, void* workspace, size_t workspace_bytes, const int* M_dev,
                      const int* N1_dev, int M_hint, void* stream);
+int d3f_gemm_x3_rowpos(const float* A, int N1, int lda, int C1, const int* idx, int ld_idx, const float* skip, int lds, int C2,
+                       const void* Wx, float* C, int ldc, int M, int N, const float* row_scale, const float* col_scale,
+                       const float* col_shift, const float* residual, int ldr, int leaky, float alpha, void* workspace,
+                       size_t workspace_bytes, const int* M_dev, const int* N1_dev, int M_hint, unsigned char* row_pos, void* stream);
+int d3f_gemm_x3_gres_rowpos(const float* A, int N1, int lda, int C1, const int* idx, int ld_idx, const float* skip, int lds, int C2,
+                            const void* Wx, float* C, int ldc, int M, int N, const float* row_scale, const float* col_scale,
+                            const float* col_shift, const float* residual, int ldr, const int* res_idx, int ld_res_idx, int res_rows,
+                            const int* res_rows_dev, int leaky, float alpha, void* workspace, size_t workspace_bytes, const int* M_dev,
+                            const int* N1_dev, int M_hint, unsigned char* row_pos, void* stream);
 
 size_t d3f_gemm_bf16_workspace_bytes(int M, int N, int K, int M_hint);
 int d3f_gemm_pack_bf16(const float* W, int ldb, int K, int N, void* W_packed, void* stream);
```

Result: no change. 1954 fragments/s, median of 6 (+0.7%).
